# MobilityFirst/gigapaxos

Hardware: AMD Instinct MI355X
Metric: decided_ops_per_sec (higher is better)
Workload: dtype int32; 1 GPU; BASELINE config #3: 1000000 Paxos groups x 3 replicas per GPU, synthetic shuffled accept-reply stream; step = propose_batch(G) + accept_reply_batch(K*G votes), inputs resident in HBM; groups_per_gpu=1000000, groups_total=1000000, replicas=3, rounds_seeded_individually=96, ordered_proposals_promise=True, ordered_batches_mask=1, parallelism=groups sharded across GPUs, no collective on the decide path

## Files before the change

### gigapaxos_amd/csrc/gpx_ar16.hip.h

```cpp
#pragma once
#include "gpx_kernels.hip.h"
#include "gpx_tiles.hip.h"

struct __attribute__((aligned(16))) Vote16 {
  int32_t idx, slot, maxcp;
  uint32_t meta;
};
#define V16_LG_MASK 0x3fffu
#define V16_ESC 0x4000u
#define V16_MAX_SHIFT 10
#define GPX_TL_BUCKET_DYN_MAX (152 * 1024)

struct Stage16 {
  int32_t* base;
  int64_t n;
  __host__ __device__ __forceinline__ int32_t* gidx() const { return base; }
  __host__ __device__ __forceinline__ int32_t* slot() const { return base + n; }
  __host__ __device__ __forceinline__ int32_t* bnum() const { return base + 2 * n; }
  __host__ __device__ __forceinline__ int32_t* bcoord() const { return base + 3 * n; }
  __host__ __device__ __forceinline__ int32_t* median() const { return base + 4 * n; }
  __host__ __device__ __forceinline__ uint8_t* kind() const { return (uint8_t*)(base + 5 * n); }
};
struct VoteCols {
  const int32_t *bnum, *bcoord, *acceptor;
// ... 190 lines not shown
      const bool esc = (meta & V16_ESC) != 0;
      out.bnum = esc ? in.bnum[ix] : b0n;
      out.bcoord = esc ? in.bcoord[ix] : b0c;
    } else {
      out.c = cp;
      if (meta & V16_ESC) {
        out.b = in.acceptor[ix];
        out.bnum = in.bnum[ix];
        out.bcoord = in.bcoord[ix];
      } else {
        out.b = (int32_t)(meta >> 16);
        out.bnum = b0n;
        out.bcoord = b0c;
      }
    }
    done++;
    return true;
  }
  __device__ __forceinline__ void emit(int32_t slot, int32_t x, int32_t y, int32_t z, int32_t kind) {
    if (AC) {
      slot = x;
      z = y;
    }
    if (LDSM) {
      slotA[cur] = slot;
      cpA[cur] = z;
      metaA[cur] = (uint32_t)kind;
      if (nib)
        omask |= 1u << (done - 1);
      else
        keys[nout] = cur;
    } else {
      recG[cur].slot = slot;
      recG[cur].maxcp = z;
      recG[cur].meta = (uint32_t)kind;
      keys[nout] = cur;
    }
    nout++;
  }
  __device__ __forceinline__ void output(int32_t q, int32_t* slot, int32_t* median, int32_t* kind,
                                         uint32_t* om) const {
    uint32_t p;
    if (LDSM && nib) {
      const int d = __ffs((int)*om) - 1;
      *om &= *om - 1;
      p = (uint32_t)start + (uint32_t)stride * (uint32_t)((order >> (4 * d)) & 15ull);
    } else {
      p = (uint32_t)keys[q];
    }
    if (LDSM) {
      *slot = slotA[p];
      *median = cpA[p];
      *kind = (int32_t)metaA[p];
    } else {
      *slot = recG[p].slot;
      *median = recG[p].maxcp;
      *kind = (int32_t)recG[p].meta;
    }
  }
};

__device__ __forceinline__ unsigned long long arrival_order(const int32_t* idxA, int32_t start, int32_t c, int32_t stride = 1) {
  unsigned long long order = 0;
  if (c <= 4) {
    const uint32_t inf = 0xffffffffu;
    const uint32_t i0 = (uint32_t)idxA[start];
    const uint32_t i1 = c > 1 ? (uint32_t)idxA[start + stride] : inf;
    const uint32_t i2 = c > 2 ? (uint32_t)idxA[start + 2 * stride] : inf;
    const uint32_t i3 = c > 3 ? (uint32_t)idxA[start + 3 * stride] : inf;
    const uint32_t r0 = (i1 < i0) + (i2 < i0) + (i3 < i0);
    const uint32_t r1 = (i0 < i1) + (i2 < i1) + (i3 < i1);
    const uint32_t r2 = (i0 < i2) + (i1 < i2) + (i3 < i2);
    const uint32_t r3 = 6u - r0 - r1 - r2;
    const uint32_t o = (1u << (4 * r1)) | (2u << (4 * r2)) | (3u << (4 * r3));
    order = o & 0xffffu;
  } else {
    for (int32_t t = 0; t < c; t++) {
      const uint32_t it = (uint32_t)idxA[start + t * stride];
      int32_t r = 0;
      for (int32_t u = 0; u < c; u++) r += (uint32_t)idxA[start + u * stride] < it;
      order |= (unsigned long long)t << (4 * r);
    }
  }
  return order;
}

#ifdef GPX_AR16_WAVES
#define GPX_AR16_ATTR __attribute__((amdgpu_waves_per_eu(GPX_AR16_WAVES, 8)))
#else
#define GPX_AR16_ATTR
#endif
struct AcceptOut {
  int32_t *r_bnum, *r_bcoord, *r_maxcp;
  uint8_t* r_flags;
  I4* r_packed;
};
#define B16_AR 0
#define B16_ACCEPT 1
#define B16_COMMIT 2
template <int OP, int KMAX, class IT>
__device__ __forceinline__ void ar16_replay_group(const DevState& S, const DevScratch& X, int32_t g, IT& it, CoordPre<KMAX>& P,
                                                  const VoteCols& in, const AcceptOut& R, uint8_t* __restrict__ status,
                                                  const int32_t* idxA, int32_t* slotA, int32_t* cpA, uint32_t* metaA,
                                                  int32_t start, int32_t pstride, int32_t c) {
  auto replay = [&](auto& it_) {
    if (OP == B16_AR)
      apply_ar_group<KMAX>(S, X, g, it_, status, P);
    else if (OP == B16_ACCEPT)
      apply_accept_group(S, X, g, it_, R.r_bnum, R.r_bcoord, R.r_maxcp, R.r_flags, status, R.r_packed);
    else
      apply_commit_group(S, X, g, it_, status);
  };
  if (it.nib) it.order = arrival_order(idxA, start, c, pstride);
  bool fast = false;
  int32_t s0 = 0;
  uint32_t skip = 0;
  int32_t nvote = c;
  bool esc = false;
  if (OP == B16_AR) {
    const bool idle = (P.gf & (GF_EXISTS | GF_STOPPED | GF_HASCOORD)) == GF_EXISTS;
    bool el = c <= 8 && (P.gf & (GF_EXISTS | GF_STOPPED | GF_HASCOORD | GF_PREPARING)) == (GF_EXISTS | GF_HASCOORD) &&
              it.b0n == P.my_bnum && it.b0c == P.my_bcoord;
    if (idle) {
      el = true;
      nvote = 0;
    } else if (el) {
      bool have = false;
      for (int32_t i = 0; i < c; i++) {
        const uint32_t p = (uint32_t)start + (uint32_t)pstride * (uint32_t)((it.order >> (4 * i)) & 15ull);
        if (metaA[p] & V16_ESC) {
          esc = true;
          const int32_t ix = idxA[p];
          const int32_t cmp = ballot_cmp(in.bnum[ix], in.bcoord[ix], P.my_bnum, P.my_bcoord);
          if (cmp < 0) {
            skip |= 1u << i;
            continue;
          }
          el = el && cmp == 0;
        }
        const int32_t sl = slotA[p];
        if (!have) s0 = sl;
        have = true;
        el = el && sl == s0;
      }
      if (have) {
        const int32_t d = jsub(P.next, s0);
        el = el && d >= 1 && d <= S.W;
      }
    }
    fast = __all(el);
  }
  if (fast) {
    if (OP == B16_AR) {
      const int32_t G = S.G, k = (int32_t)GF_K(P.gf);
      int32_t mem[KMAX], ns[KMAX];
#pragma unroll
      for (int j = 0; j < KMAX; j++) {
        mem[j] = (j < k) ? P.mem[j] : 0;
        ns[j] = (j < k) ? P.ns[j] : 0;
      }
      const int64_t off = (int64_t)(s0 & (S.W - 1)) * G + g;
      const uint32_t e0 = (P.have_pe && s0 == jsub(P.next, 1)) ? P.pe : S.p_ring[off];
      uint32_t e = e0;
      int32_t pcount = P.pcount;
      bool ns_dirty = false;
      auto vote = [&](int32_t i, uint32_t p, int32_t acc, int32_t maxcp) {
        int32_t midx = -1;
#pragma unroll
        for (int q = 0; q < KMAX; q++) {
          if (q < k && mem[q] == acc) {
            midx = q;
            if (ns[q] < maxcp) {
              ns[q] = maxcp;
              ns_dirty = true;
            }
          }
        }
        if (e & PR_PRESENT) {
          if (midx >= 0) e |= (1u << midx);
          if (__popc(e & 0xffffu) > k / 2) {
            slotA[p] = s0;
            cpA[p] = median_minus<KMAX>(ns, k);
            metaA[p] = (uint32_t)GPX_D_DECISION;
            it.omask |= 1u << i;
            it.nout++;
            e = 0;
            pcount--;
          }
        }
      };
      if (!__any(esc)) {
        for (int32_t i = 0; i < nvote; i++) {
          const uint32_t p = (uint32_t)start + (uint32_t)pstride * (uint32_t)((it.order >> (4 * i)) & 15ull);
          vote(i, p, (int32_t)(metaA[p] >> 16), cpA[p]);
        }
      } else {
        for (int32_t i = 0; i < nvote; i++) {
          if ((skip >> i) & 1u) continue;
          const uint32_t p = (uint32_t)start + (uint32_t)pstride * (uint32_t)((it.order >> (4 * i)) & 15ull);
          const uint32_t meta = metaA[p];
          vote(i, p, (meta & V16_ESC) ? in.acceptor[idxA[p]] : (int32_t)(meta >> 16), cpA[p]);
        }
      }
      if (e != e0) S.p_ring[off] = e;
      if (ns_dirty) {
#pragma unroll
        for (int q = 0; q < KMAX; q++)
          if (q < k) S.node_slots[(int64_t)q * G + g] = ns[q];
      }
      if (pcount != P.pcount) S.c_pcount[g] = pcount;
    }
  } else {
    replay(it);
  }
}

struct TileLds {
  int32_t* pre;
  uint16_t* st;
};
#define GPX_TILE_LDS_DECL(TILES_)                                   \
  __shared__ int32_t s_pre_[(TILES_) ? GPX_TL_MAXWG + 1 : 1];       \
  __shared__ uint16_t s_st_[(TILES_) ? GPX_TL_MAXWG : 1];           \
  const TileLds TL{s_pre_, s_st_}
template <int OP, int KMAX, bool TILES = false>
__device__ __forceinline__ void bucket16_body(const DevState& S, const DevScratch& X, const Stage16& O, const VoteCols& in,
                                              const AcceptOut& R, uint8_t* __restrict__ status, const TileLds& TL,
                                              const TileArea& A = TileArea{}, int32_t b_in = -1,
                                              const PlaceCols& IP = PlaceCols{}) {
  extern __shared__ __attribute__((aligned(16))) int32_t lds[];
  constexpr bool AC = OP != B16_AR;
  if ((AC || X.gate) && *X.unsorted != X.epoch) return;
  int32_t b = b_in >= 0 ? b_in : (int32_t)blockIdx.x;
  if (TILES && A.xcd_rows && b_in < 0) {
    b = tile_of_block(X.nbk);
    if (b >= X.nbk) return;
  }
  const int32_t gb = X.gb;
  const int32_t l = (int32_t)threadIdx.x;
  int32_t boff, nb;
  int32_t* const s_pre = TL.pre;
  uint16_t* const s_st = TL.st;
  if (TILES) TL_STAMP(4096 + b, 0);
  if (TILES) {
    const unsigned long long* r0 = (const unsigned long long*)A.off + (uint32_t)(b >> 2) * (uint32_t)A.nwg_pad;
    const unsigned long long* r1 = (const unsigned long long*)A.off + (uint32_t)((b + 1) >> 2) * (uint32_t)A.nwg_pad;
    const int32_t per = (A.nwg + gb - 1) >> X.shift;
    int32_t cw[4], ssum = 0, csum = 0;
#pragma unroll
    for (int q = 0; q < 4; q++) {
      const int32_t w = l * per + q;
      cw[q] = 0;
      if (q < per && w < A.nwg) {
        const unsigned long long e0 = r0[w];
        const unsigned long long e1 = ((b & 3) == 3) ? r1[w] : e0;
        const uint16_t o0 = (uint16_t)(e0 >> (16 * (b & 3))), o1 = (uint16_t)(e1 >> (16 * ((b + 1) & 3)));
        const int32_t st = (int32_t)(o0 & 0x7fffu);
        cw[q] = (int32_t)(o1 & 0x7fffu) - st;
        s_st[w] = o0;
        ssum += st;
        csum += cw[q];
      }
    }
    int32_t ex = block_exscan_and_sum_rt(csum, ssum, &nb, &boff);
#pragma unroll
    for (int q = 0; q < 4; q++) {
      const int32_t w = l * per + q;
      if (q < per && w < A.nwg) {
        s_pre[w] = ex;
        ex += cw[q];
      }
    }
    if (l == 0) {
      s_pre[A.nwg] = nb;
      X.bucket_off[b] = boff;
      if (nb == 0) X.bucket_nout[b] = 0;
    }
  } else {
    boff = X.bucket_off[b];
    nb = X.bucket_off[b + 1] - boff;
    if (threadIdx.x == 0) {
      X.bucket_tot[b] = 0;
      if (nb == 0) X.bucket_nout[b] = 0;
    }
  }
  if (nb == 0) return;
  const int32_t g = X.g_base + (b << X.shift) + l;
#ifdef GPX_B16_NOPRELOAD
  const bool pre = false;
#else
  const bool pre = !AC && 2 * nb >= gb;
#endif
  CoordPre<KMAX> P;
  P.have_pe = false;
  P.my_bnum = P.my_bcoord = 0;
  if (pre && g < X.g_end) coord_preload<KMAX>(S, g, P);
  const int32_t L = X.lds_recs;
  int32_t* lcnt = lds;
  int32_t* lcur = lds + gb;
  int32_t* idxA = lds + 2 * gb;
  int32_t* slotA = idxA + L;
  int32_t* cpA = slotA + L;
  uint32_t* metaA = (uint32_t*)(cpA + L);
  const bool in_lds = nb <= L;
  Vote16* recG = (Vote16*)X.rec + boff;
  unsigned long long* keysG = X.perm + boff;
  lcnt[l] = 0;
  const int32_t slot0 = TILES ? A.ref[0] : 0;
  const int32_t ref_bn = TILES ? A.ref[1] : in.bnum[0], ref_bc = TILES ? A.ref[2] : in.bcoord[0];
  int32_t ip_pb = 0, ip_span = -1;
  if (TILES && !AC && IP.div) {
    ip_pb = IP.quot(boff);
    ip_span = IP.quot(boff + nb) - ip_pb;
  }
  int32_t srch = 0;
  if (TILES)
    while ((1 << srch) < A.nwg) srch++;
  auto tile_find = [&](int32_t j) -> int32_t {
    int32_t lo = 0, hi = A.nwg;
    for (int32_t t = 0; t < srch; t++) {
      const int32_t mid = (lo + hi) >> 1;
      const bool up = s_pre[mid] <= j;
      lo = up ? mid : lo;
      hi = up ? hi : mid;
    }
    return lo;
  };
  auto tile_adv = [&](int32_t j, int32_t lo) -> int32_t {
    while (s_pre[lo + 1] <= j) lo++;
    return lo;
  };
  auto tile_pos = [&](int32_t j, int32_t lo, uint32_t* wide) -> uint32_t {
    const uint32_t st = s_st[lo];
    *wide = st & TL_WIDE;
    return __umul24((uint32_t)lo, (uint32_t)A.tile) + (st & 0x7fffu) + (uint32_t)(j - s_pre[lo]);
  };
  auto tile_exp = [&](const Vote8 raw, uint32_t p, uint32_t wide, int32_t lo) -> Vote16 {
    const I4 x = tile_expand(raw, wide ? A.ext + p : (const int2*)nullptr, lo, A.tile, slot0, in.slot, in.maxcp);
    Vote16 v;
    v.idx = x.x, v.slot = x.y, v.maxcp = x.z, v.meta = (uint32_t)x.w;
    return v;
  };
  auto tile_at = [&](int32_t j, int32_t lo) -> Vote16 {
    uint32_t wide;
    const uint32_t p = tile_pos(j, lo, &wide);
    return tile_exp(A.recs[p], p, wide, lo);
  };
  auto tile_rec = [&](int32_t j) -> Vote16 { return tile_at(j, tile_find(j)); };
  if (TILES) __syncthreads();
  if (TILES) TL_STAMP(4096 + b, 1);
#ifdef GPX_ABL_STOP
  if (TILES && GPX_ABL_STOP == 1) return;
#endif
  if (TILES && !in_lds) {
    for (int32_t j = l; j < nb; j += gb) recG[j] = tile_rec(j);
    __threadfence_block();
  }
  __syncthreads();
  Vote16 r0, r1, r2, r3;
  r0.meta = r1.meta = r2.meta = r3.meta = 0;
  r0.idx = r1.idx = r2.idx = r3.idx = 0;
  r0.slot = r1.slot = r2.slot = r3.slot = 0;
  r0.maxcp = r1.maxcp = r2.maxcp = r3.maxcp = 0;
// ... 177 lines not shown
      }
      O.kind()[o] = (uint8_t)kd;
    }
  };
  auto in_place = [&](int32_t tout) -> int32_t {
    if (!TILES || AC || !IP.div) return -1;
    if (tout == ip_span) return ip_pb;
    if (l == 0) A.ref[3] = (int32_t)X.epoch;
    return -1;
  };
  auto put_in_place = [&](int32_t o, int32_t a, int32_t z, int32_t kd) {
    IP.gidx[o] = g;
    IP.slot[o] = a;
    IP.median[o] = z;
    IP.bnum[o] = P.my_bnum;
    IP.bcoord[o] = P.my_bcoord;
    IP.kind[o] = (uint8_t)kd;
  };
  if (in_lds) {
    VoteIter<true, AC> it;
    it.idxA = idxA;
    it.slotA = slotA;
    it.cpA = cpA;
    it.metaA = metaA;
    it.recG = recG;
    it.keys = keysG + start;
    it.in = in;
    it.b0n = ref_bn;
    it.b0c = ref_bc;
    it.start = start;
    it.stride = pstride;
    it.c = c;
    it.done = 0;
    it.nout = 0;
    it.nib = c <= V16_NIB_MAX;
    it.order = 0;
    it.omask = 0;
    it.cur = 0;
    if (live) ar16_replay_group<OP, KMAX>(S, X, g, it, P, in, R, status, idxA, slotA, cpA, metaA, start, pstride, c);
    nout = it.nout;
    omask = it.omask;
    if (TILES) TL_STAMP(4096 + b, 4);
#ifdef GPX_ABL_STOP
    if (TILES && GPX_ABL_STOP == 3) return;
#endif
    int32_t tout;
    const int32_t ex = block_exscan_rt(nout, &tout);
    const int32_t pb = in_place(tout);
    for (int32_t q = 0; q < nout; q++) {
      int32_t sl, md, kd;
      it.output(q, &sl, &md, &kd, &omask);
      put((int64_t)boff + ex + q, sl, md, kd);
      if (pb >= 0) put_in_place(pb + ex + q, sl, md, kd);
    }
    if (l == 0) X.bucket_nout[b] = tout;
    if (TILES) TL_STAMP(4096 + b, 5);
  } else {
    VoteIter<false, AC> it;
    it.idxA = idxA;
    it.slotA = slotA;
    it.cpA = cpA;
    it.metaA = metaA;
    it.recG = recG;
    it.keys = keysG + start;
    it.in = in;
    it.b0n = ref_bn;
    it.b0c = ref_bc;
    it.start = start;
    it.stride = 1;
    it.c = c;
    it.done = 0;
    it.nout = 0;
    it.nib = false;
    it.order = 0;
    it.omask = 0;
    it.cur = 0;
    if (live) replay(it);
    nout = it.nout;
    int32_t tout;
    const int32_t ex = block_exscan_rt(nout, &tout);
    const int32_t pb = in_place(tout);
    for (int32_t q = 0; q < nout; q++) {
      int32_t sl, md, kd;
      it.output(q, &sl, &md, &kd, &omask);
      put((int64_t)boff + ex + q, sl, md, kd);
      if (pb >= 0) put_in_place(pb + ex + q, sl, md, kd);
    }
    if (l == 0) X.bucket_nout[b] = tout;
  }
}

template <int OP, int KMAX>
__global__ __launch_bounds__(1024) GPX_AR16_ATTR void k_bucket16(DevState S, DevScratch X, Stage16 O, VoteCols in,
                                                   AcceptOut R, uint8_t* __restrict__ status) {
  GPX_TILE_LDS_DECL(false);
  bucket16_body<OP, KMAX>(S, X, O, in, R, status, TL);
}
struct TilesKernArgs {
  DevState S;
  DevScratch X;
  Stage16 O;
  VoteCols in;
  uint8_t* status;
  TileArea A;
  PlaceCols IP;
};
static_assert(alignof(DevState) == 8 && alignof(DevScratch) == 8 && alignof(Stage16) == 8 && alignof(VoteCols) == 8 &&
                  alignof(TileArea) == 8 && alignof(PlaceCols) == 8,
              "kernarg layout");
static_assert(sizeof(DevState) % 8 == 0 && sizeof(DevScratch) % 8 == 0 && sizeof(Stage16) % 8 == 0 && sizeof(VoteCols) % 8 == 0 &&
                  sizeof(TileArea) % 8 == 0 && sizeof(PlaceCols) % 8 == 0,
              "kernarg layout");
#ifndef GPX_LAZY
#define GPX_LAZY 7
#endif
template <bool LAZY, class T>
__device__ __forceinline__ const T& lazy_pick(const T& from_kernarg, const T& by_value) {
  if constexpr (LAZY) return from_kernarg;
  else return by_value;
}
#define GPX_TILES_KERNEL_BODY(KM)                                                                                          \
  GPX_TILE_LDS_DECL(true);                                                                                                 \
  const TilesKernArgs* ka = (const TilesKernArgs*)__builtin_amdgcn_kernarg_segment_ptr();                                  \
  bucket16_body<B16_AR, KM, true>(lazy_pick<(GPX_LAZY & 16) != 0>(ka->S, S), lazy_pick<(GPX_LAZY & 2) != 0>(ka->X, X), O,  \
                                  lazy_pick<(GPX_LAZY & 1) != 0>(ka->in, in), AcceptOut{},                                 \
                                  (GPX_LAZY & 8) ? ka->status : status, TL, lazy_pick<(GPX_LAZY & 32) != 0>(ka->A, A), -1, \
                                  lazy_pick<(GPX_LAZY & 4) != 0>(ka->IP, IP))
template <int KMAX>
__global__ __launch_bounds__(1024) GPX_AR16_ATTR void k_bucket_ar16_tiles(DevState S, DevScratch X, Stage16 O, VoteCols in,
                                                                         uint8_t* __restrict__ status, TileArea A, PlaceCols IP) {
  GPX_TILES_KERNEL_BODY(KMAX);
}
#ifndef GPX_K4_WAVES
#define GPX_K4_WAVES 6
#endif
__global__ __launch_bounds__(1024) __attribute__((amdgpu_waves_per_eu(GPX_K4_WAVES, 8))) void k_bucket_ar16_tiles_k4(
    DevState S, DevScratch X, Stage16 O, VoteCols in, uint8_t* __restrict__ status, TileArea A, PlaceCols IP) {
  GPX_TILES_KERNEL_BODY(4);
}
__global__ __launch_bounds__(1024) __attribute__((amdgpu_waves_per_eu(6, 8))) void k_bucket_ar16_tiles_k5(
    DevState S, DevScratch X, Stage16 O, VoteCols in, uint8_t* __restrict__ status, TileArea A, PlaceCols IP) {
  GPX_TILES_KERNEL_BODY(5);
}
__global__ __launch_bounds__(1024) __attribute__((amdgpu_waves_per_eu(6, 8))) void k_bucket_ar16_k5(
    DevState S, DevScratch X, Stage16 O, VoteCols in, AcceptOut R, uint8_t* __restrict__ status) {
  GPX_TILE_LDS_DECL(false);
  bucket16_body<B16_AR, 5>(S, X, O, in, R, status, TL);
}

__global__ __launch_bounds__(GPX_BLOCK) void k_emit_dec16(
    DevScratch X, Stage16 O, int32_t* __restrict__ d_gidx, int32_t* __restrict__ d_slot,
    int32_t* __restrict__ d_bnum, int32_t* __restrict__ d_bcoord, int32_t* __restrict__ d_median,
    uint8_t* __restrict__ d_kind, int32_t* total_out, unsigned long long* acc, const int32_t* base_in,
    int32_t* chain_out, int32_t* in_place = nullptr, int32_t nvotes = 0, const int32_t* __restrict__ c_bnum = nullptr,
    const int32_t* __restrict__ c_bcoord = nullptr) {
  if (X.gate && *X.unsorted != X.epoch) return;
  const bool placed = in_place && in_place[3] != (int32_t)X.epoch;
  if (placed && blockIdx.x != gridDim.x - 1) return;
  const int32_t base0 = base_in ? *base_in : 0;
  const int32_t b = blockIdx.x;
  int32_t before = 0;
  for (int32_t t = threadIdx.x; t < b; t += GPX_BLOCK) before += X.bucket_nout[t];
  int32_t pre;
  block_exscan(before, &pre);
  const int32_t out0 = base0 + pre;
  if (b == (int32_t)gridDim.x - 1 && threadIdx.x == 0) {
    const int32_t tot = pre + X.bucket_nout[b];
    if (total_out) *total_out = base0 + tot;
    if (chain_out) *chain_out = base0 + tot;
    if (acc) atomicAdd(acc, (unsigned long long)tot);
    if (in_place && !placed && tot > 0 && nvotes % tot == 0 && nvotes / tot <= 64 && X.xabort)
      __hip_atomic_store(X.xabort + GPX_IP_LEARN_WORD, (uint32_t)(nvotes / tot), __ATOMIC_RELAXED, __HIP_MEMORY_SCOPE_SYSTEM);
    if (in_place) in_place[placed ? 5 : 6]++;
  }
  if (placed) return;
  const int32_t nd = X.bucket_nout[blockIdx.x];
  const int64_t src = X.bucket_off[blockIdx.x];
  if (threadIdx.x == 0) X.bucket_tot[blockIdx.x] = 0;
  for (int32_t t = threadIdx.x; t < nd; t += GPX_BLOCK) {
    const int32_t g = O.gidx()[src + t];
    d_gidx[out0 + t] = g;
    d_slot[out0 + t] = O.slot()[src + t];
    d_bnum[out0 + t] = c_bnum ? c_bnum[g] : O.bnum()[src + t];
    d_bcoord[out0 + t] = c_bnum ? c_bcoord[g] : O.bcoord()[src + t];
    d_median[out0 + t] = O.median()[src + t];
    d_kind[out0 + t] = O.kind()[src + t];
  }
}

__global__ __launch_bounds__(GPX_BLOCK) void k_emit_runs16(DevScratch X, Stage16 O, int32_t* __restrict__ x_gidx,
                                                          int32_t* __restrict__ x_first,
                                                          int32_t* __restrict__ x_count, int32_t* total_out) {
  if (*X.unsorted != X.epoch) return;
  const int32_t out0 = emit_base(X, total_out, nullptr);
  const int32_t nd = X.bucket_nout[blockIdx.x];
  const int64_t src = X.bucket_off[blockIdx.x];
  for (int32_t t = threadIdx.x; t < nd; t += GPX_BLOCK) {
    x_gidx[out0 + t] = O.gidx()[src + t];
    x_first[out0 + t] = O.slot()[src + t];
    x_count[out0 + t] = O.median()[src + t];
  }
}

__global__ __launch_bounds__(GPX_BLOCK) void k_unpack_replies(DevScratch X, int32_t n, const I4* __restrict__ rows,
                                                             int32_t* __restrict__ r_bnum,
                                                             int32_t* __restrict__ r_bcoord,
                                                             int32_t* __restrict__ r_maxcp,
                                                             uint8_t* __restrict__ r_flags) {
  if (*X.unsorted != X.epoch) return;
  const int32_t i = blockIdx.x * GPX_BLOCK + threadIdx.x;
  if (i >= n) return;
  const I4 r = rows[i];
  r_bnum[i] = r.x;
  r_bcoord[i] = r.y;
  r_maxcp[i] = r.z;
  r_flags[i] = (uint8_t)r.w;
}
```

### gigapaxos_amd/csrc/gpx_elect.hip.h

```cpp
#pragma once

struct PReplyIn {
  const int32_t* pv_off;
  int32_t pv_total;
  const int32_t *pv_slot, *pv_bnum, *pv_bcoord;
  const int64_t* pv_handle;
  const uint8_t* pv_flags;
};
struct PReplyOut {
  int32_t n;
  uint8_t* v_kind;
  int32_t *e_count, *e_median, *e_slot;
  uint8_t* e_kind;
  int64_t* e_handle;
  uint8_t* e_flags;
  uint8_t* status;
};

__global__ __launch_bounds__(GPX_BLOCK) void k_election_begin(DevState S, int32_t n,
                                                             const int32_t* __restrict__ gidx,
                                                             const int32_t* __restrict__ bnum,
                                                             uint8_t* __restrict__ e_status) {
  const int32_t i = blockIdx.x * GPX_BLOCK + threadIdx.x;
  if (i >= n) return;
  const int32_t g = gidx[i];
  if ((uint32_t)g >= (uint32_t)S.G || !(S.g_flags[g] & GF_EXISTS)) {
    e_status[i] = 255;
    return;
  }
  const uint32_t gf = S.g_flags[g];
  const int32_t k = (int32_t)GF_K(gf);
  const bool has = (gf & GF_HASCOORD) != 0;
  const int32_t cmp = has ? ballot_cmp(S.c_bnum[g], S.c_bcoord[g], bnum[i], S.my_id) : -1;
  if (!has || cmp < 0) {
    S.c_bnum[g] = bnum[i];
    S.c_bcoord[g] = S.my_id;
    S.c_next[g] = S.a_slot[g];
    S.c_pcount[g] = 0;
    S.c_wait[g] = 0;
    for (int32_t j = 0; j < k; j++) S.node_slots[(int64_t)j * S.G + g] = -1;
    for (int32_t w = 0; w < S.W; w++) {
      const int64_t o = (int64_t)w * S.G + g;
      S.p_ring[o] = 0;
      S.co_ring[o] = I4{0, 0, 0, 0};
    }
    if (bnum[i] == 0) {
      S.g_flags[g] = (gf | GF_HASCOORD) & ~GF_PREPARING;
      e_status[i] = GPX_EB_ACTIVE;
    } else {
      S.g_flags[g] = gf | GF_HASCOORD | GF_PREPARING;
      e_status[i] = GPX_EB_PREPARING;
    }
  } else if (cmp == 0 && (gf & GF_PREPARING)) {
    e_status[i] = GPX_EB_RESEND;
  } else {
    e_status[i] = GPX_EB_UNCHANGED;
  }
}

template <int KMAX>
__global__ __launch_bounds__(GPX_BLOCK) void k_poke_scan(DevState S, int32_t n,
                                                        const int32_t* __restrict__ gidx,
                                                        uint8_t* __restrict__ poke,
                                                        int32_t* __restrict__ slot,
                                                        int32_t* __restrict__ bnum,
                                                        int32_t* __restrict__ bcoord,
                                                        int32_t* __restrict__ median_cp,
                                                        uint8_t* __restrict__ p_flags,
                                                        uint32_t* __restrict__ heard,
                                                        uint8_t* __restrict__ status) {
  const int32_t i = blockIdx.x * GPX_BLOCK + threadIdx.x;
  if (i >= n) return;
  const int32_t g = gidx ? gidx[i] : i;
  uint8_t pk = GPX_POKE_NONE, fl = 0, st = GPX_S_OK;
  int32_t sl = 0, bn = 0, bc = 0, med = 0;
  uint32_t hd = 0;
  if ((uint32_t)g >= (uint32_t)S.G || !(S.g_flags[g] & GF_EXISTS)) {
    st = GPX_S_NOGROUP;
  } else {
    const uint32_t gf = S.g_flags[g];
    if (gf & GF_HASCOORD) {
      const int32_t s = S.a_slot[g];
      if (gf & GF_PREPARING) {
        pk = GPX_POKE_PREPARE;
        hd = S.c_wait[g];
      } else {
        const int32_t d = jsub(S.c_next[g], s);
        const uint32_t e = (d >= 1 && d <= S.W) ? S.p_ring[(int64_t)(s & (S.W - 1)) * S.G + g] : 0u;
        if (e & PR_PRESENT) {
          const int32_t k = (int32_t)GF_K(gf);
          int32_t ns[KMAX];
#pragma unroll
          for (int q = 0; q < KMAX; q++) ns[q] = (q < k) ? S.node_slots[(int64_t)q * S.G + g] : 0;
          pk = GPX_POKE_ACCEPT;
          med = median_minus<KMAX>(ns, k);
          fl = (e & PR_STOP) ? GPX_PV_STOP : 0;
          hd = e & 0xffffu;
        }
      }
      if (pk != GPX_POKE_NONE) {
        sl = s;
        bn = S.c_bnum[g];
        bc = S.c_bcoord[g];
      }
    }
  }
  poke[i] = pk;
  slot[i] = sl;
  bnum[i] = bn;
  bcoord[i] = bc;
  median_cp[i] = med;
  p_flags[i] = fl;
  heard[i] = hd;
  status[i] = st;
}

#define FE_PRESENT 0x1000u
#define FE_STOP 0x1u
#define FE_KIND(e) (((e) >> 4) & 0xfu)
#define FE_MAKE(kind, stop) (FE_PRESENT | ((uint32_t)(kind) << 4) | ((stop) ? FE_STOP : 0u))

template <class F>
__device__ __forceinline__ void for_signed_order(int32_t lo, int32_t cnt, F f) {
  if (cnt <= 0) return;
  const int32_t hi = (int32_t)((uint32_t)lo + (uint32_t)(cnt - 1));
  int32_t split = 0;
  if (hi < lo) split = (int32_t)(0x80000000u - (uint32_t)lo);
  for (int32_t j = split; j < cnt; j++) f(j);
  for (int32_t j = 0; j < split; j++) f(j);
}

#ifdef GPX_ELECT_BOUNDS
#define EI(i) elect_idx((int32_t)(i), WMAX, __LINE__)
__device__ __forceinline__ int32_t elect_idx(int32_t i, int32_t lim, int line) {
  if ((uint32_t)i >= (uint32_t)lim) {
    printf("elect_group: index %d outside [0, %d) at gpx_elect.hip.h:%d\n", i, lim, line);
    __builtin_trap();
  }
  return i;
}
#else
#define EI(i) (i)
#endif
template <int KMAX, int WMAX>
#ifdef GPX_ELECT_NOINLINE
#define GPX_ELECT_INLINE __attribute__((noinline))
#else
#define GPX_ELECT_INLINE __forceinline__
#endif
__device__ GPX_ELECT_INLINE void elect_group(const DevState& S, const DevScratch& X, int32_t g,
                                         GroupIter& it, const PReplyIn& I, const PReplyOut& O) {
  const int32_t G = S.G, W = S.W, Wm = W - 1, n = O.n;
  uint32_t gf = S.g_flags[g];
  const uint32_t gf0 = gf;
  const bool exists = (gf & GF_EXISTS) != 0;
  const int32_t k = (int32_t)GF_K(gf);
  const bool had = exists && (gf & GF_HASCOORD);
  const int32_t my_bnum = had ? S.c_bnum[g] : 0, my_bcoord = had ? S.c_bcoord[g] : 0;
  int32_t next = had ? S.c_next[g] : 0, pcount = had ? S.c_pcount[g] : 0;
  uint32_t wait = (had && (gf & GF_PREPARING)) ? S.c_wait[g] : 0u;
  int32_t mem[KMAX], ns[KMAX];
#pragma unroll
  for (int q = 0; q < KMAX; q++) {
    mem[q] = (had && q < k) ? S.members[(int64_t)q * G + g] : 0;
    ns[q] = (had && q < k) ? S.node_slots[(int64_t)q * G + g] : 0;
  }
  bool ns_dirty = false, wait_dirty = false, prop_dirty = false;
  int32_t cs[WMAX], cb[WMAX], cc[WMAX], cf[WMAX];
  int64_t ch[WMAX];
  bool co_loaded = false;
  unsigned long long cmask = 0, co_dirty = 0;
  unsigned long long n_drop = 0;

  auto list_preactives = [&](int32_t ix) -> int32_t {
    int32_t cnt = 0;
    const int32_t lo = jsub(next, pcount);
    for_signed_order(lo, pcount, [&](int32_t j) {
      const int32_t s = (int32_t)((uint32_t)lo + (uint32_t)j);
      const int64_t o = (int64_t)(s & Wm) * G + g;
      const uint32_t pe = S.p_ring[o];
      const int64_t q = (int64_t)cnt * n + ix;
      O.e_slot[q] = s;
      O.e_kind[q] = GPX_E_PREACTIVE;
      O.e_handle[q] = S.p_handle[o];
      O.e_flags[q] = (pe & PR_STOP) ? GPX_PV_STOP : 0;
      cnt++;
    });
    return cnt;
  };

  Rec r;
  while (it.next(r)) {
    const int32_t ix = r.idx, acceptor = r.a, first = r.b;
    uint8_t vk = GPX_V_IGNORED;
    int32_t ecount = 0, emed = 0;
    if (!exists) {
      O.status[ix] = GPX_S_NOGROUP;
      n_drop++;
    } else if ((gf & GF_HASCOORD) && (gf & GF_PREPARING)) {
      const int32_t cmp = ballot_cmp(r.bnum, r.bcoord, my_bnum, my_bcoord);
      if (cmp > 0) {
        ecount = list_preactives(ix);
        for (int32_t d = 1; d <= pcount; d++) S.p_ring[(int64_t)(jsub(next, d) & Wm) * G + g] = 0;
        pcount = 0;
        prop_dirty = true;
        gf &= ~(GF_HASCOORD | GF_PREPARING);
        vk = GPX_V_PREEMPTED;
      } else if (cmp == 0) {
        int32_t midx = -1;
#pragma unroll
        for (int q = 0; q < KMAX; q++)
          if (q < k && mem[q] == acceptor) midx = q;
        if (midx >= 0 && !((wait >> midx) & 1u)) {
          if (!co_loaded) {
            for (int32_t w = 0; w < W; w++) {
              const I4 v = S.co_ring[(int64_t)w * G + g];
              cs[EI(w)] = v.x;
              cb[EI(w)] = v.y;
              cc[EI(w)] = v.z;
              cf[EI(w)] = v.w;
              ch[EI(w)] = S.co_handle[(int64_t)w * G + g];
              if (v.w & CO_PRESENT) cmask |= 1ull << w;
            }
            co_loaded = true;
          }
          const int32_t o = I.pv_off[ix], m = I.pv_off[ix + 1] - o;
          bool clash = o < 0 || m < 0 || (int64_t)o + m > (int64_t)I.pv_total;
          if (!clash) {
            int32_t claimed[WMAX];
            unsigned long long nm = 0;
            for (int32_t j = 0; j < m; j++) {
              const int32_t s = I.pv_slot[o + j], x = s & Wm;
              if ((nm >> x) & 1ull) {
                if (claimed[EI(x)] != s) clash = true;
              } else if (((cmask >> x) & 1ull) && cs[EI(x)] != s) {
                clash = true;
              }
              claimed[EI(x)] = s;
              nm |= 1ull << x;
            }
          }
          if (clash) {
            O.status[ix] = GPX_S_WINDOW;
            n_drop++;
          } else {
            vk = GPX_V_RECORDED;
            int32_t ms = first;
            for (int32_t j = 0; j < m; j++) {
              const int32_t s = I.pv_slot[o + j];
              if (jsub(s, ms) < 0) ms = s;
            }
#pragma unroll
            for (int q = 0; q < KMAX; q++)
              if (q < k && mem[q] == acceptor && jsub(ns[q], ms) < 0) {
                ns[q] = ms;
                ns_dirty = true;
              }
            for (int32_t j = 0; j < m; j++) {
              const int32_t s = I.pv_slot[o + j], x = s & Wm;
              const int32_t bn = I.pv_bnum[o + j], bc = I.pv_bcoord[o + j];
              if (!((cmask >> x) & 1ull) || ballot_cmp(bn, bc, cb[EI(x)], cc[EI(x)]) > 0) {
                cs[EI(x)] = s;
                cb[EI(x)] = bn;
                cc[EI(x)] = bc;
                cf[EI(x)] = CO_PRESENT | (I.pv_flags ? (int32_t)(I.pv_flags[o + j] & (GPX_PV_STOP | GPX_PV_NOOP)) : 0);
                ch[EI(x)] = I.pv_handle ? I.pv_handle[o + j] : 0;
                cmask |= 1ull << x;
                co_dirty |= 1ull << x;
              }
            }
            wait |= 1u << midx;
            wait_dirty = true;
            if (__popc(wait & 0xffffu) > k / 2) {
              uint32_t fe[WMAX];
              int64_t fh[WMAX];
              bool fits = true;
              int32_t lo = jsub(next, pcount), pos = pcount;
              if (cmask == 0) {
                ecount = list_preactives(ix);
              } else {
                int32_t maxCarry = 0, maxMin = ns[0];
                bool any = false;
                for (int32_t w = 0; w < W; w++)
                  if ((cmask >> w) & 1ull) {
                    if (!any || jsub(cs[EI(w)], maxCarry) > 0) maxCarry = cs[EI(w)];
                    any = true;
                  }
#pragma unroll
                for (int q = 0; q < KMAX; q++)
                  if (q < k && jsub(ns[q], maxMin) > 0) maxMin = ns[q];
                const int32_t R = jsub(maxCarry, maxMin);
                if (R >= W || R == INT32_MIN) {
                  fits = false;
                } else {
                  const int32_t pre_lo = jsub(next, pcount);
                  unsigned long long removed = 0;
                  bool stop_exists = false, last_stop = false;
                  lo = R >= 0 ? maxMin : (int32_t)((uint32_t)maxCarry + 1u);
                  pos = 0;
                  for (int32_t j = 0; j <= R; j++) {
                    const int32_t cur = (int32_t)((uint32_t)maxMin + (uint32_t)j), x = cur & Wm;
                    const int32_t d = jsub(cur, pre_lo);
                    uint32_t en = 0;
                    int64_t hn = 0;
                    if (((cmask >> x) & 1ull) && cs[EI(x)] == cur) {
                      en = FE_MAKE(GPX_E_CARRY, cf[EI(x)] & GPX_PV_STOP);
                      hn = ch[EI(x)];
                    } else if (!(d >= 0 && d < pcount)) {
                      en = FE_MAKE(GPX_E_NOOP, 0);
                    } else {
                      const int64_t po = (int64_t)x * G + g;
                      const uint32_t pe = S.p_ring[po];
                      const int64_t ph = S.p_handle[po];
                      bool dup = false;
                      for (int32_t w = 0; w < W; w++) dup |= ((cmask >> w) & 1ull) && ch[EI(w)] == ph;
                      if (!dup) {
                        en = FE_MAKE(GPX_E_PREACTIVE, pe & PR_STOP);
                        hn = ph;
                      }
                      removed |= 1ull << d;
                    }
                    fe[EI(pos)] = en;
                    fh[EI(pos)] = hn;
                    if (en & FE_PRESENT) {
                      stop_exists |= (en & FE_STOP) != 0;
                    }
                    last_stop = (en & FE_PRESENT) && (en & FE_STOP);
                    pos++;
                  }
                  auto append = [&](uint32_t en, int64_t hn) {
                    if (pos > 0 && last_stop) return;
                    if (pos < W) {
                      fe[EI(pos)] = en;
                      fh[EI(pos)] = hn;
                    }
                    pos++;
                    stop_exists |= (en & FE_STOP) != 0;
                    last_stop = (en & FE_STOP) != 0;
                  };
                  for_signed_order(pre_lo, pcount, [&](int32_t dd) {
                    if ((removed >> dd) & 1ull) return;
                    const int32_t s = (int32_t)((uint32_t)pre_lo + (uint32_t)dd);
                    const int64_t po = (int64_t)(s & Wm) * G + g;
                    append(FE_MAKE(GPX_E_PREACTIVE, S.p_ring[po] & PR_STOP), S.p_handle[po]);
                  });
                  if (stop_exists && pos > 0 && !last_stop) append(FE_MAKE(GPX_E_NEWSTOP, 1), 0);
                  fits = pos <= W;
                  if (fits) {
                    for (int32_t d = 1; d <= pcount; d++) S.p_ring[(int64_t)(jsub(next, d) & Wm) * G + g] = 0;
                    int32_t live = 0;
                    for (int32_t j = 0; j < pos; j++)
                      if (fe[EI(j)] & FE_PRESENT) {
                        const int32_t s = (int32_t)((uint32_t)lo + (uint32_t)j);
                        S.p_ring[(int64_t)(s & Wm) * G + g] = PR_PRESENT | ((fe[EI(j)] & FE_STOP) ? PR_STOP : 0u);
                        live++;
                      }
                    next = (int32_t)((uint32_t)lo + (uint32_t)pos);
                    pcount = live;
                    prop_dirty = true;
                    for_signed_order(lo, pos, [&](int32_t j) {
                      if (!(fe[EI(j)] & FE_PRESENT)) return;
                      const int64_t q = (int64_t)ecount * n + ix;
                      O.e_slot[q] = (int32_t)((uint32_t)lo + (uint32_t)j);
                      O.e_kind[q] = (uint8_t)FE_KIND(fe[EI(j)]);
                      O.e_handle[q] = fh[EI(j)];
                      O.e_flags[q] = (fe[EI(j)] & FE_STOP) ? GPX_PV_STOP : 0;
                      ecount++;
                    });
                  }
                }
              }
              if (fits) {
                emed = median_minus<KMAX>(ns, k);
                gf &= ~GF_PREPARING;
                vk = GPX_V_ELECTED;
              } else {
                O.status[ix] = GPX_S_WINDOW;
                n_drop++;
              }
            }
          }
        }
      }
    }
    O.v_kind[ix] = vk;
    O.e_count[ix] = ecount;
    O.e_median[ix] = emed;
  }
  if (co_dirty) {
    for (int32_t w = 0; w < W; w++)
      if ((co_dirty >> w) & 1ull) {
        S.co_ring[(int64_t)w * G + g] = I4{cs[EI(w)], cb[EI(w)], cc[EI(w)], cf[EI(w)]};
        S.co_handle[(int64_t)w * G + g] = ch[EI(w)];
      }
  }
  if (ns_dirty) {
#pragma unroll
    for (int q = 0; q < KMAX; q++)
      if (q < k) S.node_slots[(int64_t)q * G + g] = ns[q];
  }
  if (wait_dirty) S.c_wait[g] = wait;
  if (prop_dirty) {
    S.c_next[g] = next;
    S.c_pcount[g] = pcount;
  }
  if (gf != gf0) S.g_flags[g] = gf;
  if (n_drop) atomicAdd(&X.counters[2], n_drop);
}

template <int KMAX, int WMAX>
__global__ __launch_bounds__(1024) void k_bucket_prepare_reply(DevState S, DevScratch X, PReplyIn I,
                                                               PReplyOut O) {
  extern __shared__ __attribute__((aligned(16))) int32_t lds[];
  BucketView bv;
  if (!bucket_prepare(X, lds, &bv, []() {})) return;
  const int32_t g0 = blockIdx.x << X.shift;
  for (int32_t l = threadIdx.x; l < X.gb; l += (int32_t)blockDim.x) {
    const int32_t c = bv.lcnt[l];
    const int32_t g = g0 + l;
    if (c == 0 || g >= S.G) continue;
    GroupIter it;
    it.init(bv, l, c);
    elect_group<KMAX, WMAX>(S, X, g, it, I, O);
  }
}
```

### gigapaxos_amd/csrc/gpx_engine.hip

```cpp
#include <hip/hip_runtime.h>
#include <unistd.h>
#include <dirent.h>
#include <signal.h>
#include <sys/stat.h>
#include <sys/types.h>
#include <cerrno>
#include <chrono>

#include <cmath>
#include <cstdio>
#include <cstdlib>
#include <cstring>
#include <map>
#include <mutex>
#include <string>
#include <vector>
#include <algorithm>
#include <cassert>
#include <initializer_list>

#include "gpx_kernels.hip.h"
#include "gpx_ar16.hip.h"
#include "gpx_direct.hip.h"
#include "gpx_one.hip.h"
// ... 413 lines not shown
    LAUNCH_F(e, "k_hist", k_hist<true>, tile_grid(nsuper), lds, n, ntiles, gidx, e->S.G, e->X, status,
             is_votes, check_order, hsub);
  else
    LAUNCH_F(e, "k_hist", k_hist<false>, tile_grid(nsuper), lds, n, ntiles, gidx, e->S.G, e->X, status,
             is_votes, check_order, hsub);
}

void launch_scatter_ac(gpx_engine* e, int32_t n, const int32_t* gidx, const int32_t* bnum,
                       const int32_t* bcoord, const int32_t* slot, const int32_t* median_cp,
                       const uint8_t* flags, int32_t* r_bnum, int32_t* r_bcoord, int32_t* r_maxcp,
                       uint8_t* r_flags, int32_t only_unsorted = 0) {
  const int ntiles = ntiles_for(n);
  const bool vec = aligned16({gidx, bnum, bcoord, slot, median_cp}) && !((uintptr_t)flags & 3);
  if (vec)
    LAUNCH_F(e, "k_scatter_ac", k_scatter_ac<true>, tile_grid(ntiles), (size_t)e->X.nbk * 4, n, ntiles,
             e->S.G, e->X, gidx, bnum, bcoord, slot, median_cp, flags, r_bnum, r_bcoord, r_maxcp, r_flags,
             only_unsorted);
  else
    LAUNCH_F(e, "k_scatter_ac", k_scatter_ac<false>, tile_grid(ntiles), (size_t)e->X.nbk * 4, n, ntiles,
             e->S.G, e->X, gidx, bnum, bcoord, slot, median_cp, flags, r_bnum, r_bcoord, r_maxcp, r_flags,
             only_unsorted);
}

int check_batch(gpx_engine* h, int32_t n) {
  if (!h || n < 0) return GPX_EINVAL;
  if (n > h->cfg.max_batch) return GPX_ECAPACITY;
  if (h->h_abort && *(volatile uint32_t*)h->h_abort) {
    snprintf(g_err, sizeof(g_err), "an exchange kernel gave up waiting for its grid (call epoch %u): engine state is "
             "incomplete; set GPX_DEVICE_SHARERS to the number of processes sharing the device", *(volatile uint32_t*)h->h_abort);
    return GPX_EDEVICE;
  }
  return GPX_OK;
}

#define SYNC_CHECKED(h, stream_)                                \
  do {                                                          \
    HIPCHK(hipStreamSynchronize(stream_));                      \
    if (int _rc_abort = check_batch((h), 0)) return _rc_abort;  \
  } while (0)

int xchg_share(const gpx_engine* e) {
  std::lock_guard<std::mutex> lk(g_live_mu);
  int live = 1;
  auto it = g_live_streams.find(e->device);
  if (it != g_live_streams.end()) live = std::max<int>(1, (int)it->second.size());
  if (e->sharers_set) return live * e->sharers;
  return live + proc_registry_foreign(e->device);
}
bool xchg_ctl(gpx_engine* e, int nchunks, GridXchg* Q, int* grid, const void* kernel, int block) {
  const int g16 = (std::max(nchunks, 1) + GPX_GX_LINES - 1) / GPX_GX_LINES * GPX_GX_LINES;
  if (!e->one_launch) return false;
  int per_cu = 2;
  {
    auto it = e->occ.find(kernel);
    if (it == e->occ.end()) {
      int nb = 0;
      if (hipOccupancyMaxActiveBlocksPerMultiprocessor(&nb, kernel, block, 0) != hipSuccess) {
        (void)hipGetLastError();
        nb = 0;
      }
      it = e->occ.emplace(kernel, nb).first;
    }
    per_cu = std::min(2, it->second - 1);
  }
  if (per_cu < 1 || (int64_t)g16 * xchg_share(e) > (int64_t)per_cu * e->cus) return false;
  const OneCtl C = one_ctl(e);
  *grid = g16;
  Q->arrive = (uint32_t*)(e->one_words + GPX_ONE_TICKETS);
  Q->verdict = C.verdict;
  Q->epoch = C.epoch;
  e->gx_arrive += (uint32_t)(g16 / GPX_GX_LINES);
  Q->arrive_target = e->gx_arrive + e->xchg_test_skew;
  Q->timeout_ms = e->xchg_timeout_ms;
  return true;
}

constexpr size_t GPX_PAGEABLE_PIECE = (size_t)512 << 10;
bool host_is_pinned(gpx_engine* e, const void* p) {
  for (auto& r : e->registered)
    if ((const char*)p >= r.first && (const char*)p < r.first + r.second) return true;
  hipPointerAttribute_t at{};
  if (hipPointerGetAttributes(&at, p) != hipSuccess) {
    (void)hipGetLastError();
    return false;
  }
  return at.type == hipMemoryTypeHost;
}
hipError_t xfer(gpx_engine* e, void* dst, const void* src, size_t bytes, hipMemcpyKind kind, hipStream_t st) {
  if (bytes <= GPX_PAGEABLE_PIECE || host_is_pinned(e, kind == hipMemcpyHostToDevice ? src : (const void*)dst))
    return hipMemcpyAsync(dst, src, bytes, kind, st);
  for (size_t o = 0; o < bytes; o += GPX_PAGEABLE_PIECE) {
    const hipError_t rc = hipMemcpyAsync((char*)dst + o, (const char*)src + o, std::min(GPX_PAGEABLE_PIECE, bytes - o), kind, st);
    if (rc != hipSuccess) return rc;
  }
  return hipSuccess;
}

template <int KMAX>
void launch_bucket_ar16(gpx_engine* e, const Stage16& O, const VoteCols& in, uint8_t* status) {
  LAUNCH_B(e, "k_bucket_ar16", (k_bucket16<B16_AR, KMAX>), e->S, e->X, O, in, AcceptOut{}, status);
}
template <int KMAX>
void launch_bucket_propose(gpx_engine* e, int32_t* slot, int32_t* bnum, int32_t* bcoord,
                           int32_t* median, uint8_t* status, const int64_t* handle) {
  LAUNCH_B(e, "k_bucket_propose", (k_bucket_propose<KMAX>), e->S, e->X, slot, bnum, bcoord, median,
           status, handle);
}

struct Stage {
  gpx_engine* e;
  size_t in_off = 0, out_off = 0;
  explicit Stage(gpx_engine* e_) : e(e_) {}
  static size_t a16(size_t b) { return (b + 15) & ~(size_t)15; }
  template <typename T>
  const T* in(const T* host, size_t count) {
    if (!host) return nullptr;
    const size_t b = count * sizeof(T);
    memcpy(e->hs_in + in_off, host, b);
    const T* d = (const T*)(e->ds_in + in_off);
    in_off += a16(b);
    return d;
  }
  template <typename T>
  T* out(size_t count, const T** host_view) {
    T* d = (T*)(e->ds_out + out_off);
    *host_view = (const T*)(e->hs_out + out_off);
    out_off += a16(count * sizeof(T));
    return d;
  }
  int upload() {
    if (in_off) HIPCHK(hipMemcpyAsync(e->ds_in, e->hs_in, in_off, hipMemcpyHostToDevice, e->sF));
    return GPX_OK;
  }
  int finish() {
    HIPCHK(hipMemcpyAsync(e->hs_out, e->ds_out, out_off, hipMemcpyDeviceToHost, e->sB));
    HIPCHK(hipStreamSynchronize(e->sB));
    return check_batch(e, 0);
  }
};

}

extern "C" {

int gpx_abi_version(void) { return GPX_ABI_VERSION; }
const char* gpx_last_error(void) { return g_err; }

int gpx_engine_create(const gpx_config* cfg, gpx_engine** out) {
  g_err[0] = 0;
  if (!cfg || !out) return GPX_EINVAL;
  if (cfg->max_groups <= 0 || cfg->kmax < 1 || cfg->kmax > GPX_KMAX_LIMIT || cfg->max_batch <= 0)
    return GPX_EINVAL;
  if (cfg->window < 4 || cfg->window > 64 || (cfg->window & (cfg->window - 1))) return GPX_EINVAL;
  int ndev = 0;
  hipError_t de = hipErrorNoDevice;
  const int attempts = access("/dev/kfd", F_OK) == 0 ? 15 : 1;
  for (int attempt = 0; attempt < attempts; attempt++) {
    de = hipGetDeviceCount(&ndev);
    if (de == hipSuccess && ndev > 0) break;
    (void)hipGetLastError();
    if (de != hipErrorNoDevice && de != hipSuccess) break;
    if (attempt + 1 < attempts) usleep(200 * 1000);
  }
  if (de != hipSuccess || ndev <= 0) {
    snprintf(g_err, sizeof(g_err), "no HIP device visible (%s)", de == hipSuccess ? "count 0" : hipGetErrorString(de));
    return GPX_EDEVICE;
  }
  gpx_engine* e = new gpx_engine();
  e->cfg = *cfg;
#define HIPCHK_CREATE(expr)                                                                  \
  do {                                                                                       \
    hipError_t _e = (expr);                                                                  \
    if (_e != hipSuccess) {                                                                  \
      snprintf(g_err, sizeof(g_err), "%s:%d %s -> %s", __FILE__, __LINE__, #expr,            \
               hipGetErrorString(_e));                                                       \
      gpx_engine_destroy(e);                                                                 \
      return GPX_EDEVICE;                                                                    \
    }                                                                                        \
  } while (0)
  if (cfg->device >= 0) {
    HIPCHK_CREATE(hipSetDevice(cfg->device));
    e->device = cfg->device;
  } else {
    HIPCHK_CREATE(hipGetDevice(&e->device));
  }
  HIPCHK_CREATE(hipStreamCreateWithFlags(&e->own_stream, hipStreamNonBlocking));
  apply_streams(e);
  const size_t G = (size_t)cfg->max_groups, W = (size_t)cfg->window, K = (size_t)cfg->kmax;
  const size_t N = (size_t)cfg->max_batch;
  DevState& S = e->S;
  S.G = cfg->max_groups;
  S.kmax = cfg->kmax;
  S.W = cfg->window;
  S.my_id = cfg->my_id;
  S.flags = cfg->flags;
  int rc = GPX_OK;
#define A(ptr, count, zero)                                   \
  if ((rc = dev_alloc(e, &(ptr), (count), (zero))) != GPX_OK) { \
    gpx_engine_destroy(e);                                    \
    return rc;                                                \
  }
  A(S.g_flags, G, true);
  A(S.g_version, G, true);
  A(S.a_slot, G, true);
  A(S.a_bnum, G, true);
  A(S.a_bcoord, G, true);
  A(S.a_gc, G, true);
  A(S.c_bnum, G, true);
  A(S.c_bcoord, G, true);
  A(S.c_next, G, true);
  A(S.c_pcount, G, true);
  A(S.members, K * G, true);
  A(S.node_slots, K * G, true);
  A(S.p_ring, W * G, true);
  A(S.acc_ring, W * G, true);
  A(S.com_ring, W * G, true);
  DevScratch& X = e->X;
  auto nbk_for = [&](int sh) { return (int64_t)((G + ((size_t)1 << sh) - 1) >> sh); };
  X.shift = nbk_for(GPX_MIN_SHIFT + 1) >= 256 ? GPX_MIN_SHIFT + 1 : GPX_MIN_SHIFT;
  while (nbk_for(X.shift) > GPX_MAX_BUCKETS) X.shift++;
  if (const char* sh = getenv("GPX_BUCKET_SHIFT")) {
    const int v = atoi(sh);
    if (v >= GPX_MIN_SHIFT && v <= 20 && nbk_for(v) <= GPX_MAX_BUCKETS) X.shift = v;
  }
  X.gb = 1 << X.shift;
  X.nbk = (int32_t)nbk_for(X.shift);
  X.g_base = 0;
  X.g_end = cfg->max_groups;
  e->bucket_threads = std::min(1024, X.gb);
  {
    int64_t want = (int64_t)cfg->kmax * X.gb;
    want += want / 4 + 64;
    if (cfg->kmax <= 3 && X.gb == 256) want = 960;
    const int64_t lds_cap = ((int64_t)160 * 1024 - 1024 - (int64_t)X.gb * 8) / (8 + 4 * GPX_PAY_WORDS);
    want = std::min<int64_t>(want, std::min<int64_t>(lds_cap, (int64_t)GPX_BUCKET_ITEMS * e->bucket_threads));
    if (const char* lr = getenv("GPX_LDS_RECS")) want = std::min<int64_t>(want, std::max(64, atoi(lr)));
    X.lds_recs = (int32_t)want;
    e->lds_recs_max = X.lds_recs;
    e->lds_recs_hw = (int32_t)std::max<int64_t>(want, std::min<int64_t>(lds_cap, (int64_t)GPX_BUCKET_ITEMS * e->bucket_threads));
  }
  {
    const int64_t cap16 = ((int64_t)160 * 1024 - 1024 - (int64_t)X.gb * 8) / 16;
    int64_t want = (int64_t)cfg->kmax * X.gb;
    want += want / 4 + 128;
    e->lds16_max = (int32_t)std::min<int64_t>(want, cap16);
    e->lds16_hw = (int32_t)cap16;
    e->ac16 = X.shift <= V16_MAX_SHIFT && e->bucket_threads == X.gb;
    if (X.shift <= V16_MAX_SHIFT) {
      e->shift16 = X.shift;
      e->nbk16 = X.nbk;
      e->ar_passes = 1;
    } else {
      e->shift16 = V16_MAX_SHIFT;
      const int64_t range = (int64_t)GPX_MAX_BUCKETS << V16_MAX_SHIFT;
      e->ar_passes = (int32_t)(((int64_t)G + range - 1) / range);
      e->nbk16 = GPX_MAX_BUCKETS;
      const int64_t gb16 = (int64_t)1 << V16_MAX_SHIFT;
      const int64_t cap16b = ((int64_t)160 * 1024 - 1024 - gb16 * 8) / 16;
      int64_t want16 = (int64_t)cfg->kmax * gb16;
      want16 += want16 / 4 + 128;
      e->lds16_max = (int32_t)std::min<int64_t>(want16, cap16b);
      e->lds16_hw = (int32_t)cap16b;
    }
    if ((rc = dev_alloc(e, &e->ar_chain, 2, true)) != GPX_OK) {
      gpx_engine_destroy(e);
      return rc;
    }
  }
  if (const char* lp = getenv("GPX_LDS_PAD")) e->lds_pad = (size_t)std::max(0, atoi(lp));
  if (const char* tr = getenv("GPX_TRY_RUNS")) e->env_mask = atoi(tr) ? GPX_TRY_REPLY_RUNS : 0;
  e->ar_tiles = true;
  if (const char* sl = getenv("GPX_AR_TILES")) e->ar_tiles = atoi(sl) != 0;
  if (const char* sl = getenv("GPX_AR_INPLACE")) e->ar_in_place = atoi(sl) != 0;
  if (const char* tt = getenv("GPX_TILE_T")) e->tile_force = atoi(tt);
  if (const char* tt = getenv("GPX_TILE_NT")) e->tile_threads = atoi(tt);
  e->tile_area.xcd_rows = 1;
  if (const char* xr = getenv("GPX_TILE_XCD_ROWS")) e->tile_area.xcd_rows = atoi(xr) != 0;
#ifdef GPX_TL_TRACE
  if (const char* ab = getenv("GPX_TL_ABLATE")) e->tile_area.xcd_rows |= atoi(ab) << 1;
#endif
  if (const char* sv = getenv("GPX_SAR_MAX_N")) e->sar_max_n = std::max(0, std::min(GPX_SAR_MAX_N, atoi(sv)));
  e->sar_max_n = std::min(e->sar_max_n, cfg->max_batch);
  e->ordered_mask = e->env_mask;
  e->bucket_lds = GPX_BUCKET_LDS_BYTES(X.gb, X.lds_recs) + e->lds_pad;
  const size_t bucket_lds_hw = GPX_BUCKET_LDS_BYTES(X.gb, e->lds_recs_hw) + e->lds_pad;
  if (bucket_lds_hw > 64 * 1024) {
    const void* fns[] = {(const void*)k_bucket_propose<4>,
                         (const void*)k_bucket_propose<8>, (const void*)k_bucket_propose<16>,
                         (const void*)k_bucket_accept,     (const void*)k_bucket_commit,
                         (const void*)k_bucket_pack_ar,    (const void*)k_bucket_reqbatch,
                         (const void*)k_bucket_prepare,
                         (const void*)k_bucket_prepare_reply<4, 64>,
                         (const void*)k_bucket_prepare_reply<8, 64>,
                         (const void*)k_bucket_prepare_reply<16, 64>};
    for (const void* f : fns)
      HIPCHK_CREATE(hipFuncSetAttribute(f, hipFuncAttributeMaxDynamicSharedMemorySize, (int)bucket_lds_hw));
  }
  {
    if ((rc = dev_alloc(e, &e->small_tickets, 2 * (GPX_SMALL_DIRECT_MAX_N / GPX_DCHUNK), true)) != GPX_OK ||
        (rc = dev_alloc(e, &e->small_draw, 1, true)) != GPX_OK) {
      gpx_engine_destroy(e);
      return rc;
    }
    if (hipHostMalloc((void**)&e->hs_in, GPX_STAGE_BYTES, hipHostMallocDefault) != hipSuccess ||
        hipHostMalloc((void**)&e->hs_out, GPX_STAGE_BYTES, hipHostMallocDefault) != hipSuccess) {
      snprintf(g_err, sizeof(g_err), "hipHostMalloc(%zu) failed", (size_t)GPX_STAGE_BYTES);
      gpx_engine_destroy(e);
      return GPX_ENOMEM;
    }
    if ((rc = dev_alloc(e, &e->ds_in, GPX_STAGE_BYTES, false)) != GPX_OK ||
        (rc = dev_alloc(e, &e->ds_out, GPX_STAGE_BYTES, false)) != GPX_OK) {
      gpx_engine_destroy(e);
      return rc;
    }
  }
  {
    const size_t hw16 = GPX_BUCKET16_LDS_BYTES((size_t)1 << e->shift16, e->lds16_hw) + e->lds_pad;
    const void* fns[] = {(const void*)k_bucket16<B16_AR, 4>, (const void*)k_bucket_ar16_k5, (const void*)k_bucket16<B16_AR, 8>,
                         (const void*)k_bucket16<B16_AR, 16>, (const void*)k_bucket16<B16_ACCEPT, 4>,
                         (const void*)k_bucket16<B16_COMMIT, 4>};
    for (const void* f : fns)
      HIPCHK_CREATE(hipFuncSetAttribute(f, hipFuncAttributeMaxDynamicSharedMemorySize, (int)hw16));
  }
  {
    const void* fns[] = {(const void*)k_ar_tiny<4>, (const void*)k_ar_tiny<8>, (const void*)k_ar_tiny<16>};
    for (const void* f : fns)
      HIPCHK_CREATE(hipFuncSetAttribute(f, hipFuncAttributeMaxDynamicSharedMemorySize, (int)GPX_SAR_LDS_BYTES));
  }
  {
    const int hl = GPX_HSUB_MAX * std::max(X.nbk, e->nbk16) * (int)sizeof(int32_t);
    if (hl > 64 * 1024) {
      HIPCHK_CREATE(hipFuncSetAttribute((const void*)k_hist<true>, hipFuncAttributeMaxDynamicSharedMemorySize, hl));
      HIPCHK_CREATE(hipFuncSetAttribute((const void*)k_hist<false>, hipFuncAttributeMaxDynamicSharedMemorySize, hl));
    }
  }
  const size_t nbk_alloc = (size_t)std::max(X.nbk, e->nbk16);
  for (auto& f : e->fs) {
    A(f.bucket_tot, nbk_alloc, true);
    A(f.tile_rel, ((N + GPX_TILE - 1) / GPX_TILE) * nbk_alloc, false);
    A(f.bucket_off, nbk_alloc + 1, true);
    A(f.rec, N, false);
    A(f.unsorted, 1, true);
    A(f.chunk_cnt, GPX_CHUNK_CNT_WORDS(N), true);
  }
  X.bucket_tot = e->fs[0].bucket_tot;
  X.tile_rel = e->fs[0].tile_rel;
  X.bucket_off = e->fs[0].bucket_off;
  X.rec = e->fs[0].rec;
  X.unsorted = e->fs[0].unsorted;
  X.epoch = 1;
  A(X.rank2, N, false);
  A(X.perm, N, false);
  A(X.o_rec, N, false);
  A(X.bucket_nout, nbk_alloc, true);
  A(e->rec_tag, N, true);
  A(e->one_words, GPX_ONE_TICKETS + GPX_GX_LINES * 16, true);
  A(X.counters, 3, true);
  for (int i = 0; i < 12; i++) A(e->st_i32[i], N, false);
  for (int i = 0; i < 4; i++) A(e->st_u8[i], N, false);
  A(e->st_count, 4, true);
#undef A
  {
    HIPCHK_CREATE(hipDeviceGetAttribute(&e->cus, hipDeviceAttributeMultiprocessorCount, e->device));
    if (const char* sv = getenv("GPX_XCHG_SLOTS")) e->one_launch = atoi(sv) != 0;
// ... 246 lines not shown
  {
    LaunchScope _ls(e, "k_route_scatter");
    hipLaunchKernelGGL(k_route_scatter, dim3(ntiles), dim3(GPX_ROUTE_NT), 0, e->stream, n, n_groups_global, n_shards,
                       C, g2l, (const int32_t*)e->route_cnt, (const int32_t*)shard_off);
  }
  HIPCHK(hipGetLastError());
  return GPX_OK;
}


struct TileShape {
  int32_t T, NT;
};
#ifdef GPX_TL_TRACE
static unsigned long long* tl_trace_dev = nullptr;
static void tl_trace_begin(gpx_engine* e) {
  if (!tl_trace_dev) {
    HIPQ(hipMalloc(&tl_trace_dev, TL_TRACE_ROWS * 8 * sizeof(unsigned long long)));
    HIPQ(hipMemcpyToSymbol(HIP_SYMBOL(g_tl_trace), &tl_trace_dev, sizeof(tl_trace_dev)));
  }
  HIPQ(hipMemsetAsync(tl_trace_dev, 0, TL_TRACE_ROWS * 8 * sizeof(unsigned long long), e->stream));
}
static void tl_trace_end(gpx_engine* e) {
  const char* tf = getenv("GPX_TL_TRACE_FILE");
  if (!tf) return;
  HIPQ(hipStreamSynchronize(e->stream));
  std::vector<unsigned long long> tr((size_t)TL_TRACE_ROWS * 8);
  HIPQ(hipMemcpy(tr.data(), tl_trace_dev, tr.size() * 8, hipMemcpyDeviceToHost));
  if (FILE* fp = fopen(tf, "wb")) {
    fwrite(tr.data(), 8, tr.size(), fp);
    fclose(fp);
  }
}
#endif
static TileShape tile_shape(const gpx_engine* e, int32_t n, int32_t nbk) {
  if (e->tile_force) return TileShape{e->tile_force, e->tile_threads ? e->tile_threads : (e->tile_force <= 8192 ? 512 : 1024)};
  const int64_t cus = std::max(1, e->cus);
  static const struct { TileShape s; int64_t round_ns; } cand[] = {{{12288, 1024}, 27900}, {{8192, 1024}, 17300}, {{4096, 512}, 10000}};
  TileShape best = cand[2].s;
  int64_t best_cost = INT64_MAX;
  for (const auto& c : cand) {
    if (GPX_TL_LDS_BYTES(nbk, c.s.T, c.s.NT) > (size_t)158 * 1024) continue;
    const int64_t nwg = ((int64_t)n + c.s.T - 1) / c.s.T;
    if (nwg > GPX_TL_MAXWG) continue;
    const int64_t cost = (nwg + cus - 1) / cus * c.round_ns + nwg * 5;
    if (cost < best_cost) best_cost = cost, best = c.s;
  }
  return best;
}
static bool ar_tiles_call(gpx_engine* e, int32_t n, const int32_t* gidx, const int32_t* bnum, const int32_t* bcoord,
                          const int32_t* slot, const int32_t* acceptor, const int32_t* max_cp, int32_t* d_gidx,
                          int32_t* d_slot, int32_t* d_bnum, int32_t* d_bcoord, int32_t* d_median_cp, uint8_t* d_kind,
                          int32_t* n_out, uint8_t* status) {
  const int32_t nbk = e->nbk16;
  if (nbk > GPX_MAX_BUCKETS || e->shift16 > 10 || e->shift16 < 8) return false;
  TileShape ts = tile_shape(e, n, nbk);
  if (nbk + 1 > ts.NT * 8) ts.NT = 1024;
  assert(nbk + 1 <= ts.NT * 8);
  const int32_t T = ts.T;
  if ((T != 4096 && T != 8192 && T != 12288 && T != 16384) || (ts.NT != 512 && ts.NT != 1024) || T % (ts.NT * 4)) return false;
  const int r4 = T / (ts.NT * 4);
  if (!(ts.NT == 1024 && r4 >= 1 && r4 <= 4) && !(ts.NT == 512 && (r4 == 2 || r4 == 4))) return false;
  if (GPX_TL_LDS_BYTES(nbk, T, ts.NT) > (size_t)158 * 1024) return false;
  const int32_t nwg = (n + T - 1) / T;
  if (nwg > GPX_TL_MAXWG) return false;
  const size_t N = (size_t)e->cfg.max_batch;
  TileArea& A = e->tile_area;
  if (!A.recs) {
    const size_t cap = (N + 4095) / 4096 * 4096 + 16384;
    const size_t nwg_max = std::min<size_t>((N + 4095) / 4096, GPX_TL_MAXWG);
    const size_t pad = (nwg_max + 7) / 8 * 8;
    if (dev_alloc(e, &A.recs, cap, false) != GPX_OK || dev_alloc(e, &A.ext, cap, false) != GPX_OK ||
        dev_alloc(e, &A.off, ((size_t)nbk / 4 + 2) * pad * 4, true) != GPX_OK || dev_alloc(e, &A.ref, 8, true) != GPX_OK) {
      A.recs = nullptr;
      e->ar_tiles = false;
      return false;
    }
    A.nwg_pad = (int32_t)pad;
    const int maxlds = (int)std::min<size_t>(GPX_TL_LDS_BYTES(nbk, 16384, 1024), (size_t)158 * 1024);
    HIPQ(hipFuncSetAttribute((const void*)k_scatter_tiles<1024, 4>, hipFuncAttributeMaxDynamicSharedMemorySize, maxlds));
    HIPQ(hipFuncSetAttribute((const void*)k_scatter_tiles<1024, 3>, hipFuncAttributeMaxDynamicSharedMemorySize, maxlds));
    HIPQ(hipFuncSetAttribute((const void*)k_scatter_tiles<1024, 2>, hipFuncAttributeMaxDynamicSharedMemorySize, maxlds));
    HIPQ(hipFuncSetAttribute((const void*)k_scatter_tiles<1024, 1>, hipFuncAttributeMaxDynamicSharedMemorySize, maxlds));
    HIPQ(hipFuncSetAttribute((const void*)k_scatter_tiles<512, 4>, hipFuncAttributeMaxDynamicSharedMemorySize, maxlds));
    HIPQ(hipFuncSetAttribute((const void*)k_scatter_tiles<512, 2>, hipFuncAttributeMaxDynamicSharedMemorySize, maxlds));
    const size_t hw16 = std::min<size_t>(GPX_BUCKET16_LDS_BYTES((size_t)1 << e->shift16, e->lds16_hw) + e->lds_pad,
                                         (size_t)GPX_TL_BUCKET_DYN_MAX);
    HIPQ(hipFuncSetAttribute((const void*)k_bucket_ar16_tiles_k4, hipFuncAttributeMaxDynamicSharedMemorySize, (int)hw16));
    HIPQ(hipFuncSetAttribute((const void*)k_bucket_ar16_tiles_k5, hipFuncAttributeMaxDynamicSharedMemorySize, (int)hw16));
    HIPQ(hipFuncSetAttribute((const void*)k_bucket_ar16_tiles<8>, hipFuncAttributeMaxDynamicSharedMemorySize, (int)hw16));
    HIPQ(hipFuncSetAttribute((const void*)k_bucket_ar16_tiles<16>, hipFuncAttributeMaxDynamicSharedMemorySize, (int)hw16));
  }
  A.nwg = nwg;
  A.tile = T;
  const DevScratch X0 = e->X;
  const int threads0 = e->bucket_threads;
  e->X.shift = e->shift16;
  e->X.gb = 1 << e->shift16;
  e->X.nbk = nbk;
  e->bucket_threads = e->X.gb;
  begin_back(e, 0, n, true);
  {
    const int32_t kslot = e->cfg.kmax <= 4 ? 4 : 8;
    if ((int64_t)n / nbk >= e->X.gb / 4 && e->X.lds_recs < kslot * e->X.gb) {
      e->X.lds_recs = kslot * e->X.gb;
      e->bucket_lds = GPX_BUCKET16_LDS_BYTES(e->X.gb, e->X.lds_recs) + e->lds_pad;
    }
  }
  if (e->bucket_lds > (size_t)GPX_TL_BUCKET_DYN_MAX) {
    e->X.lds_recs = (int32_t)(((size_t)GPX_TL_BUCKET_DYN_MAX - e->lds_pad - (size_t)e->X.gb * 8) / 16);
    e->bucket_lds = GPX_BUCKET16_LDS_BYTES(e->X.gb, e->X.lds_recs) + e->lds_pad;
  }
  const size_t lds = GPX_TL_LDS_BYTES(nbk, T, ts.NT);
#ifdef GPX_TL_TRACE
  tl_trace_begin(e);
#endif
  {
    LaunchScope _ls(e, "k_scatter_tiles");
#define GPX_LAUNCH_TILES(NT_, R4_)                                                                                       \
  hipLaunchKernelGGL(HIP_KERNEL_NAME(k_scatter_tiles<NT_, R4_>), dim3(tile_grid(A.nwg)), dim3(NT_), lds, e->stream, n, e->S.G, \
                     e->X, A, gidx, bnum, bcoord, slot, acceptor, max_cp, status)
    if (ts.NT == 1024 && r4 == 4) GPX_LAUNCH_TILES(1024, 4);
    else if (ts.NT == 1024 && r4 == 3) GPX_LAUNCH_TILES(1024, 3);
    else if (ts.NT == 1024 && r4 == 2) GPX_LAUNCH_TILES(1024, 2);
    else if (ts.NT == 1024 && r4 == 1) GPX_LAUNCH_TILES(1024, 1);
    else if (ts.NT == 512 && r4 == 4) GPX_LAUNCH_TILES(512, 4);
    else if (ts.NT == 512 && r4 == 2) GPX_LAUNCH_TILES(512, 2);
    else assert(!"k_scatter_tiles: no instantiation for this shape (refused above)");
#undef GPX_LAUNCH_TILES
  }
  const Stage16 O{(int32_t*)e->X.o_rec, (int64_t)N};
  const VoteCols in{bnum, bcoord, acceptor, slot, max_cp};
  int32_t ip_div = 0;
  if (e->ar_in_place && n < (1 << 26)) {
    const uint32_t learnt = e->h_abort ? ((volatile uint32_t*)e->h_abort)[GPX_IP_LEARN_WORD] : 0u;
    ip_div = learnt >= 1 && learnt <= 64 ? (int32_t)learnt : std::max(1, e->cfg.kmax);
  }
  const PlaceCols IP{d_gidx, d_slot, d_bnum, d_bcoord, d_median_cp, d_kind, ip_div,
                     ip_div > 1 ? (uint32_t)((1ull << 32) / (uint64_t)ip_div) + 1u : 0u};
  {
    LaunchScope _ls(e, e->cfg.kmax <= 4 ? "k_bucket_ar16_tiles_k4" : e->cfg.kmax <= 5 ? "k_bucket_ar16_tiles_k5" : "k_bucket_ar16_tiles");
    const dim3 grid(A.xcd_rows ? tile_grid(nbk) : nbk), block(e->bucket_threads);
    if (e->cfg.kmax <= 4)
      hipLaunchKernelGGL(k_bucket_ar16_tiles_k4, grid, block, e->bucket_lds, e->stream, e->S, e->X, O, in, status, A, IP);
    else if (e->cfg.kmax <= 5)
      hipLaunchKernelGGL(k_bucket_ar16_tiles_k5, grid, block, e->bucket_lds, e->stream, e->S, e->X, O, in, status, A, IP);
    else if (e->cfg.kmax <= 8)
      hipLaunchKernelGGL(k_bucket_ar16_tiles<8>, grid, block, e->bucket_lds, e->stream, e->S, e->X, O, in, status, A, IP);
    else
      hipLaunchKernelGGL(k_bucket_ar16_tiles<16>, grid, block, e->bucket_lds, e->stream, e->S, e->X, O, in, status, A, IP);
  }
  LAUNCH(e, "k_emit_dec16", k_emit_dec16, e->X.nbk, e->X, O, d_gidx, d_slot, d_bnum, d_bcoord, d_median_cp, d_kind, n_out,
         &e->X.counters[1], (const int32_t*)nullptr, (int32_t*)nullptr, ip_div ? A.ref : (int32_t*)nullptr, n,
         ip_div ? (const int32_t*)e->S.c_bnum : (const int32_t*)nullptr, (const int32_t*)e->S.c_bcoord);
#ifdef GPX_TL_TRACE
  tl_trace_end(e);
#endif
  const int32_t lds_recs = e->X.lds_recs;
  const int32_t gate = e->X.gate;
  e->X = X0;
  e->X.lds_recs = lds_recs;
  e->X.gate = gate;
  e->bucket_threads = threads0;
  return true;
}

static void ar_partition(gpx_engine* e, int32_t n, const int32_t* gidx, const int32_t* bnum, const int32_t* bcoord,
                         const int32_t* slot, const int32_t* acceptor, const int32_t* max_cp, int32_t* d_gidx,
                         int32_t* d_slot, int32_t* d_bnum, int32_t* d_bcoord, int32_t* d_median_cp,
                         uint8_t* d_kind, int32_t* n_out, uint8_t* status) {
  const int ntiles = ntiles_for(n);
  const bool vec = aligned16({gidx, bnum, bcoord, slot, acceptor, max_cp});
  const DevScratch X0 = e->X;
  const int threads0 = e->bucket_threads;
  const int64_t NB = ((int64_t)e->S.G + ((int64_t)1 << e->shift16) - 1) >> e->shift16;
  int64_t want_passes = e->ar_passes;
  {
    const double m = (double)n / (double)NB;
    const int64_t pc = (int64_t)((m + 5.0 * sqrt(m)) / (double)e->lds16_hw) + 1;
    want_passes = std::min<int64_t>(NB, std::max<int64_t>(want_passes, pc));
  }
  const int64_t bpp = (NB + want_passes - 1) / want_passes;
  const int32_t passes = (int32_t)((NB + bpp - 1) / bpp);
  if (e->ar_tiles && passes == 1 && vec && ar_tiles_call(e, n, gidx, bnum, bcoord, slot, acceptor, max_cp, d_gidx, d_slot, d_bnum,
                                                        d_bcoord, d_median_cp, d_kind, n_out, status))
    return;
  const size_t N = (size_t)e->cfg.max_batch;
  int32_t* o32 = (int32_t*)e->X.o_rec;
  const Stage16 O{o32, (int64_t)N};
  const VoteCols in{bnum, bcoord, acceptor};
  for (int32_t p = 0; p < passes; p++) {
    e->X.shift = e->shift16;
    e->X.gb = 1 << e->shift16;
    e->X.nbk = e->nbk16;
    e->bucket_threads = e->X.gb;
    if (passes > 1) {
      const int64_t range = bpp << e->shift16;
      e->X.g_base = (int32_t)(p * range);
      e->X.g_end = (int32_t)std::min<int64_t>(e->S.G, (p + 1) * range);
      e->X.nbk = (int32_t)((e->X.g_end - e->X.g_base + e->X.gb - 1) >> e->shift16);
    }
    if (p == 0) begin_back(e, 0, n / passes, true);
    front_hist(e, n, gidx, p == 0 ? status : nullptr, p == 0 ? 1 : -1, e->X.gate ? 2 : 0);
    if (vec)
      LAUNCH_F(e, "k_scatter_ar16", k_scatter_ar16<true>, tile_grid(ntiles), (size_t)e->X.nbk * 4, n,
               ntiles, e->S.G, e->X, gidx, bnum, bcoord, slot, acceptor, max_cp);
    else
      LAUNCH_F(e, "k_scatter_ar16", k_scatter_ar16<false>, tile_grid(ntiles), (size_t)e->X.nbk * 4, n,
               ntiles, e->S.G, e->X, gidx, bnum, bcoord, slot, acceptor, max_cp);
    if (e->cfg.kmax <= 4)
      launch_bucket_ar16<4>(e, O, in, status);
    else if (e->cfg.kmax <= 5)
      LAUNCH_B(e, "k_bucket_ar16", k_bucket_ar16_k5, e->S, e->X, O, in, AcceptOut{}, status);
    else if (e->cfg.kmax <= 8)
      launch_bucket_ar16<8>(e, O, in, status);
    else
      launch_bucket_ar16<16>(e, O, in, status);
    LAUNCH(e, "k_emit_dec16", k_emit_dec16, e->X.nbk, e->X, O, d_gidx, d_slot, d_bnum, d_bcoord,
           d_median_cp, d_kind, n_out, &e->X.counters[1],
           (const int32_t*)(p > 0 ? e->ar_chain + (p & 1) : nullptr),
           passes > 1 ? e->ar_chain + ((p + 1) & 1) : (int32_t*)nullptr);
    const int32_t lds_recs = e->X.lds_recs;
    const int32_t gate = e->X.gate;
    e->X = X0;
    e->X.lds_recs = lds_recs;
    e->X.gate = gate;
    e->bucket_threads = threads0;
  }
}

#ifdef GPX_SAR_TRACE
static unsigned long long* sar_trace_dev = nullptr;
static void sar_trace_begin(gpx_engine* e) {
  if (!sar_trace_dev) {
    HIPQ(hipMalloc(&sar_trace_dev, 256 * 16 * sizeof(unsigned long long)));
    HIPQ(hipMemcpyToSymbol(HIP_SYMBOL(g_sar_trace), &sar_trace_dev, sizeof(sar_trace_dev)));
  }
  HIPQ(hipMemsetAsync(sar_trace_dev, 0, 256 * 16 * sizeof(unsigned long long), e->stream));
}
static void sar_trace_end(gpx_engine* e) {
  const char* tf = getenv("GPX_SAR_TRACE_FILE");
  if (!tf) return;
  HIPQ(hipStreamSynchronize(e->stream));
  std::vector<unsigned long long> tr(256 * 16);
  HIPQ(hipMemcpy(tr.data(), sar_trace_dev, tr.size() * 8, hipMemcpyDeviceToHost));
  if (FILE* fp = fopen(tf, "wb")) {
    fwrite(tr.data(), 8, tr.size(), fp);
    fclose(fp);
  }
}
#endif

int gpx_accept_reply_batch_dev(gpx_engine* h, int32_t n, const int32_t* gidx,
                               const int32_t* bnum, const int32_t* bcoord, const int32_t* slot,
                               const int32_t* acceptor, const int32_t* max_cp, int32_t* d_gidx,
                               int32_t* d_slot, int32_t* d_bnum, int32_t* d_bcoord,
                               int32_t* d_median_cp, uint8_t* d_kind, int32_t* n_out,
                               uint8_t* status) {
  int rc = check_batch(h, n);
  if (rc != GPX_OK) return rc;
  if (n == 0) {
    HIPCHK(hipMemsetAsync(n_out, 0, sizeof(int32_t), h->sB));
    return GPX_OK;
  }
  gpx_engine* e = h;
  const int fs = begin_front(e);
  e->X.gate = 0;
  const bool runs_promised = (e->ordered_mask & GPX_ORDERED_REPLY_RUNS) != 0;
  const bool runs_try = runs_promised || (e->ordered_mask & GPX_TRY_REPLY_RUNS) != 0;
  if (!runs_promised && n <= e->sar_max_n && e->S.G <= GPX_SAR_MAX_G) {
    e->last.kind = 0;
#ifdef GPX_SAR_TRACE
    sar_trace_begin(e);
#endif
    {
      LaunchScope _ls(e, "k_ar_tiny");
#define GPX_LAUNCH_AR_TINY(KM)                                                                                          \
  hipLaunchKernelGGL(k_ar_tiny<KM>, dim3(1), dim3(GPX_SAR_BLOCK), GPX_SAR_LDS_BYTES, e->stream, e->S, e->X, n, gidx, bnum, \
                     bcoord, slot, acceptor, max_cp, d_gidx, d_slot, d_bnum, d_bcoord, d_median_cp, d_kind, n_out, status)
      if (e->cfg.kmax <= 4)
        GPX_LAUNCH_AR_TINY(4);
      else if (e->cfg.kmax <= 8)
        GPX_LAUNCH_AR_TINY(8);
      else
        GPX_LAUNCH_AR_TINY(16);
#undef GPX_LAUNCH_AR_TINY
    }
#ifdef GPX_SAR_TRACE
    sar_trace_end(e);
#endif
    end_call(e, fs);
    HIPCHK(hipGetLastError());
    return GPX_OK;
  }
  if (runs_try) {
    const size_t N = (size_t)e->cfg.max_batch;
    if (!e->runs_info && (rc = dev_alloc(e, &e->runs_info, 2, true)) != GPX_OK) return rc;
    RunsInfo* info = e->runs_info + (e->runs_seq & 1);
    RunsInfo* next_info = e->runs_info + ((e->runs_seq + 1) & 1);
    e->runs_seq++;
    const int nchunks = (n + GPX_DCHUNK - 1) / GPX_DCHUNK;
    const RunsStage st{DecCols{d_gidx, d_slot, d_bnum, d_bcoord, d_median_cp, d_kind}, e->rec_tag, e->fs[0].chunk_cnt,
                       Stage16{(int32_t*)e->X.o_rec, (int64_t)N}};
    const int32_t refuse = runs_promised ? 1 : 0;
    if (!e->runs_arrive &&
        (rc = dev_alloc(e, &e->runs_arrive,
                        (size_t)32 * (3 + N / GPX_RBLOCK / 16 + 1),
// ... 1183 lines not shown

int gpx_group_create(gpx_engine* h, int32_t n, const int32_t* gidx, const int32_t* members,
                     const uint8_t* k, const gpx_hri* rows, uint8_t* status) {
  if (!h || n < 0) return GPX_EINVAL;
  if (n == 0) return GPX_OK;
  if (!gidx || !members || !k || !rows) return GPX_EINVAL;
  const int32_t chunk = 1 << 18;
  int32_t *d_g = nullptr, *d_m = nullptr;
  uint8_t *d_k = nullptr, *d_s = nullptr;
  gpx_hri* d_r = nullptr;
  const int32_t c0 = std::min(n, chunk);
  HIPCHK(hipMalloc((void**)&d_g, (size_t)c0 * 4));
  HIPCHK(hipMalloc((void**)&d_m, (size_t)c0 * 4 * h->cfg.kmax));
  HIPCHK(hipMalloc((void**)&d_k, (size_t)c0));
  HIPCHK(hipMalloc((void**)&d_s, (size_t)c0));
  HIPCHK(hipMalloc((void**)&d_r, (size_t)c0 * sizeof(gpx_hri)));
  int rc = GPX_OK;
  for (int32_t o = 0; o < n && rc == GPX_OK; o += chunk) {
    const int32_t c = std::min(chunk, n - o);
    H2D_B(d_g, gidx + o, (size_t)c * 4);
    H2D_B(d_m, members + (size_t)o * h->cfg.kmax, (size_t)c * 4 * h->cfg.kmax);
    H2D_B(d_k, k + o, (size_t)c);
    H2D_B(d_r, rows + o, (size_t)c * sizeof(gpx_hri));
    LAUNCH(h, "k_group_create", k_group_create, grid_for(c), h->S, c, (const int32_t*)d_g,
           (const int32_t*)d_m, (const uint8_t*)d_k, (const gpx_hri*)d_r, d_s, NameCopies{h->N.rows, (uint8_t*)h->N.tab});
    if (status) D2H(status + o, d_s, (size_t)c);
    HIPCHK(hipStreamSynchronize(h->sB));
    rc = check_batch(h, 0);
  }
  (void)hipFree(d_g);
  (void)hipFree(d_m);
  (void)hipFree(d_k);
  (void)hipFree(d_s);
  (void)hipFree(d_r);
  return rc;
}

static int retire_impl(gpx_engine* h, int32_t n, const int32_t* gidx, int32_t mode, gpx_hri* rows,
                       uint8_t* status) {
  if (!h || n < 0) return GPX_EINVAL;
  if (n == 0) return GPX_OK;
  if (!gidx) return GPX_EINVAL;
  const int32_t chunk = 1 << 18;
  int32_t* d_g = nullptr;
  uint8_t* d_s = nullptr;
  gpx_hri* d_r = nullptr;
  const int32_t c0 = std::min(n, chunk);
  HIPCHK(hipMalloc((void**)&d_g, (size_t)c0 * 4));
  HIPCHK(hipMalloc((void**)&d_s, (size_t)c0));
  HIPCHK(hipMalloc((void**)&d_r, (size_t)c0 * sizeof(gpx_hri)));
  int rc = GPX_OK;
  for (int32_t o = 0; o < n && rc == GPX_OK; o += chunk) {
    const int32_t c = std::min(chunk, n - o);
    H2D_B(d_g, gidx + o, (size_t)c * 4);
    LAUNCH(h, "k_group_retire", k_group_retire, grid_for(c), h->S, c, (const int32_t*)d_g, mode, d_r,
           d_s, NameCopies{h->N.rows, (uint8_t*)h->N.tab});
    if (rows) D2H(rows + o, d_r, (size_t)c * sizeof(gpx_hri));
    if (status) D2H(status + o, d_s, (size_t)c);
    HIPCHK(hipStreamSynchronize(h->sB));
    rc = check_batch(h, 0);
  }
  (void)hipFree(d_g);
  (void)hipFree(d_s);
  (void)hipFree(d_r);
  return rc;
}

int gpx_group_retire(gpx_engine* h, int32_t n, const int32_t* gidx, int32_t mode, gpx_hri* rows,
                     uint8_t* status) {
  if (mode != GPX_RETIRE_PAUSE && mode != GPX_RETIRE_KILL) return GPX_EINVAL;
  return retire_impl(h, n, gidx, mode, rows, status);
}

int gpx_group_snapshot(gpx_engine* h, int32_t n, const int32_t* gidx, gpx_hri* rows,
                       uint8_t* status) {
  if (!rows) return GPX_EINVAL;
  return retire_impl(h, n, gidx, 2, rows, status);
}

int gpx_group_dump(gpx_engine* h, int32_t gidx, int32_t* buf, int32_t cap) {
  if (!h || !buf) return GPX_EINVAL;
  SYNC_CHECKED(h, h->sB);
  std::vector<int32_t> w;
  const DevState& S = h->S;
  auto rd32 = [&](const void* base, int64_t idx, int32_t* out) -> hipError_t {
    return hipMemcpy(out, (const char*)base + idx * 4, 4, hipMemcpyDeviceToHost);
  };
  if (gidx < 0 || gidx >= S.G) {
    if (cap < 1) return GPX_ECAPACITY;
    buf[0] = 0;
    return 1;
  }
  int32_t gf_i = 0;
  HIPCHK(rd32(S.g_flags, gidx, &gf_i));
  const uint32_t gf = (uint32_t)gf_i;
  w.push_back((gf & GF_EXISTS) ? 1 : 0);
  if (gf & GF_EXISTS) {
    const int32_t k = (int32_t)GF_K(gf);
    int32_t v = 0;
    HIPCHK(rd32(S.g_version, gidx, &v));
    w.push_back(v);
    w.push_back(k);
    for (int j = 0; j < k; j++) {
      HIPCHK(rd32(S.members, (int64_t)j * S.G + gidx, &v));
      w.push_back(v);
    }
    const void* accf[4] = {S.a_slot, S.a_bnum, S.a_bcoord, S.a_gc};
    for (auto p : accf) {
      HIPCHK(rd32(p, gidx, &v));
      w.push_back(v);
    }
    w.push_back((gf & GF_STOPPED) ? 1 : 0);
    struct Ent {
      int32_t slot, a, b, c;
      uint8_t f;
    };
    auto read_ring = [&](const I4* ring, int shift, std::vector<Ent>& out) -> int {
      for (int32_t x = 0; x < S.W; x++) {
        I4 fe;
        HIPCHK(hipMemcpy(&fe, S.acc_ring + ((int64_t)x * S.G + gidx), sizeof(I4), hipMemcpyDeviceToHost));
        const uint8_t f = (uint8_t)(((uint32_t)fe.w >> shift) & 0xffu);
        if (!(f & RF_PRESENT)) continue;
        I4 r = fe;
        if (ring != S.acc_ring)
          HIPCHK(hipMemcpy(&r, ring + ((int64_t)x * S.G + gidx), sizeof(I4), hipMemcpyDeviceToHost));
        out.push_back(Ent{r.x, r.y, r.z, r.w, f});
      }
      std::sort(out.begin(), out.end(), [](const Ent& p, const Ent& q) { return p.slot < q.slot; });
      return GPX_OK;
    };
    std::vector<Ent> acc, com;
    int rc = read_ring(S.acc_ring, 0, acc);
    if (rc != GPX_OK) return rc;
    rc = read_ring(S.com_ring, CF_SHIFT, com);
    if (rc != GPX_OK) return rc;
    w.push_back((int32_t)acc.size());
    for (auto& en : acc) {
      w.push_back(en.slot);
      w.push_back(en.a);
      w.push_back(en.b);
      w.push_back((en.f & RF_STOP) ? 1 : 0);
    }
    w.push_back((int32_t)com.size());
    for (auto& en : com) {
      w.push_back(en.slot);
      w.push_back(en.a);
      w.push_back(en.b);
      w.push_back(en.c);
      w.push_back((en.f & RF_HASVALUE) ? 1 : 0);
      w.push_back((en.f & RF_STOP) ? 1 : 0);
    }
    w.push_back((gf & GF_HASCOORD) ? 1 : 0);
    if (gf & GF_HASCOORD) {
      int32_t next = 0;
      HIPCHK(rd32(S.c_bnum, gidx, &v));
      w.push_back(v);
      HIPCHK(rd32(S.c_bcoord, gidx, &v));
      w.push_back(v);
      HIPCHK(rd32(S.c_next, gidx, &next));
      w.push_back(next);
      for (int j = 0; j < k; j++) {
        HIPCHK(rd32(S.node_slots, (int64_t)j * S.G + gidx, &v));
        w.push_back(v);
      }
      std::vector<std::pair<int32_t, uint32_t>> props;
      for (int32_t d = S.W; d >= 1; d--) {
        const int32_t s = (int32_t)((uint32_t)next - (uint32_t)d);
        int32_t ev = 0;
        HIPCHK(rd32(S.p_ring, (int64_t)(s & (S.W - 1)) * S.G + gidx, &ev));
        if ((uint32_t)ev & PR_PRESENT) props.push_back({s, (uint32_t)ev});
      }
      std::sort(props.begin(), props.end(),
                [](const std::pair<int32_t, uint32_t>& p, const std::pair<int32_t, uint32_t>& q) {
                  return p.first < q.first;
                });
      w.push_back((int32_t)props.size());
      for (auto& pr : props) {
        w.push_back(pr.first);
        w.push_back((pr.second & PR_STOP) ? 1 : 0);
        w.push_back((int32_t)(pr.second & 0xffffu));
      }
      const bool preparing = (gf & GF_PREPARING) != 0;
      w.push_back(preparing ? 0 : 1);
      if (preparing) {
        auto rd64 = [&](const int64_t* base, int64_t idx, int64_t* out) -> hipError_t {
          return hipMemcpy(out, base + idx, 8, hipMemcpyDeviceToHost);
        };
        w.push_back(1);
        HIPCHK(rd32(S.c_wait, gidx, &v));
        w.push_back(v);
        for (auto& pr : props) {
          int64_t hv = 0;
          HIPCHK(rd64(S.p_handle, (int64_t)(pr.first & (S.W - 1)) * S.G + gidx, &hv));
          w.push_back((int32_t)(uint32_t)hv);
          w.push_back((int32_t)((uint64_t)hv >> 32));
        }
        struct Co {
          I4 v;
          int64_t hv;
        };
        std::vector<Co> cos;
        for (int32_t x = 0; x < S.W; x++) {
          Co c;
          HIPCHK(hipMemcpy(&c.v, S.co_ring + ((int64_t)x * S.G + gidx), sizeof(I4), hipMemcpyDeviceToHost));
          if (!(c.v.w & CO_PRESENT)) continue;
          HIPCHK(rd64(S.co_handle, (int64_t)x * S.G + gidx, &c.hv));
          cos.push_back(c);
        }
        std::sort(cos.begin(), cos.end(), [](const Co& p, const Co& q) { return p.v.x < q.v.x; });
        w.push_back((int32_t)cos.size());
        for (auto& c : cos) {
          w.push_back(c.v.x);
          w.push_back(c.v.y);
          w.push_back(c.v.z);
          w.push_back(c.v.w & (GPX_PV_STOP | GPX_PV_NOOP));
          w.push_back((int32_t)(uint32_t)c.hv);
          w.push_back((int32_t)((uint64_t)c.hv >> 32));
        }
      }
    }
  }
  if ((int32_t)w.size() > cap) return GPX_ECAPACITY;
  memcpy(buf, w.data(), w.size() * sizeof(int32_t));
  return (int32_t)w.size();
}

}

#include "gpx_wire_host.inc"
#include "gpx_elect_host.inc"
```

### gigapaxos_amd/csrc/gpx_kernels.hip.h

```cpp
#pragma once
#include <hip/hip_runtime.h>
#include <stdint.h>

#include "../../include/gpx.h"

#ifdef GPX_SAR_TRACE
__device__ unsigned long long* g_sar_trace = nullptr;
#define SAR_STAMP(wg, k)                                                                             \
  do {                                                                                               \
    if (threadIdx.x == 0 && g_sar_trace) g_sar_trace[(size_t)(wg) * 16 + (k)] = wall_clock64();        \
  } while (0)
#else
#define SAR_STAMP(wg, k) do { } while (0)
#endif

#ifdef GPX_TL_TRACE
__device__ unsigned long long* g_tl_trace = nullptr;
#define TL_TRACE_ROWS 8192
#define TL_STAMP(row, k)                                                                             \
  do {                                                                                               \
    if (threadIdx.x == 0 && g_tl_trace) g_tl_trace[(size_t)(row) * 8 + (k)] = wall_clock64();          \
  } while (0)
#define TL_CLOCK(row, k)  \
  do {                                                                                               \
    if (threadIdx.x == 0 && g_tl_trace) g_tl_trace[(size_t)(row) * 8 + (k)] = clock64();               \
  } while (0)
#else
#define TL_STAMP(row, k) do { } while (0)
#define TL_CLOCK(row, k) do { } while (0)
#endif

struct __attribute__((aligned(16))) I4 {
  int32_t x, y, z, w;
};
__host__ __device__ __forceinline__ I4 mk4(int32_t x, int32_t y, int32_t z, int32_t w) {
  I4 r;
  r.x = x;
  r.y = y;
  r.z = z;
  r.w = w;
  return r;
}
struct __attribute__((aligned(32))) Rec {
  int32_t idx, lg, a, b, c, bnum, bcoord, pad;
};
struct __attribute__((aligned(32))) Out {
  int32_t gidx, slot, x, y, z, kind, pad0, pad1;
};
__device__ __forceinline__ Out mk_out(int32_t gidx, int32_t slot, int32_t x, int32_t y, int32_t z,
                                      int32_t kind) {
  Out o;
  o.gidx = gidx;
  o.slot = slot;
  o.x = x;
  o.y = y;
  o.z = z;
  o.kind = kind;
  o.pad0 = 0;
  o.pad1 = 0;
  return o;
}

#define GPX_BLOCK 256
#ifndef GPX_FBLOCK
#define GPX_FBLOCK 1024
#endif
#ifndef GPX_TILE
#define GPX_TILE 4096
#endif
#define GPX_HSUB_MAX 8
#define GPX_TILE_ITEMS (GPX_TILE / GPX_FBLOCK)
#define GPX_TILE_VECS (GPX_TILE_ITEMS / 4)
#define GPX_SCAN_ITEMS 8
#define GPX_SCAN_TILE (GPX_FBLOCK * GPX_SCAN_ITEMS)
#define GPX_SMALL_SEG 16
#define GPX_MIN_SHIFT 8
#define GPX_MAX_BUCKETS 4096

#define GF_EXISTS 1u
#define GF_STOPPED 2u
#define GF_HASCOORD 4u
#define GF_PREPARING 8u
#define GF_K(f) (((f) >> 8) & 0xffu)

#define PR_PRESENT 0x10000u
#define PR_STOP 0x20000u
#define RF_PRESENT 1
#define RF_STOP 2
#define RF_HASVALUE 4

struct DevState {
  int32_t G, kmax, W, my_id;
  uint32_t flags;
  uint32_t* g_flags;
  int32_t* g_version;
  int32_t *a_slot, *a_bnum, *a_bcoord, *a_gc;
  int32_t *c_bnum, *c_bcoord, *c_next, *c_pcount;
  int32_t* members;
  int32_t* node_slots;
  uint32_t* p_ring;
  I4* acc_ring;
  I4* com_ring;
  uint32_t* c_wait;
  I4* co_ring;
  int64_t* co_handle;
  int64_t* p_handle;
};
#define CO_PRESENT 0x100

struct DevScratch {
  int32_t shift, nbk, gb;
  int32_t g_base, g_end;
  int32_t lds_recs;
  int32_t* bucket_tot;
  int32_t* tile_rel;
  int32_t* bucket_off;
  Rec* rec;
  int32_t* rank2;
  unsigned long long* perm;
  Out* o_rec;
  int32_t* bucket_nout;
  unsigned long long* counters;
  uint32_t* unsorted;
  uint32_t epoch;
  int32_t gate;
  uint32_t* xabort;
};

#define GPX_XCHG_TIMEOUT_MS 10000u
struct XchgWait {
  uint32_t spins = 0;
  unsigned long long t0 = 0;
  __device__ __forceinline__ bool tired(uint32_t limit_ms) {
    if ((++spins & 1023u) != 0) return false;
    const unsigned long long now = wall_clock64();
    if (!t0) {
      t0 = now;
      return false;
    }
    return now - t0 > (unsigned long long)limit_ms * 100000ull;
  }
};
__device__ __forceinline__ void xchg_abort(const DevScratch& X) {
  if (X.xabort) __hip_atomic_store(X.xabort, X.epoch ? X.epoch : 1u, __ATOMIC_RELAXED, __HIP_MEMORY_SCOPE_SYSTEM);
}

__device__ __forceinline__ int32_t jsub(int32_t a, int32_t b) {
  return (int32_t)((uint32_t)a - (uint32_t)b);
}
__device__ __forceinline__ int32_t ballot_cmp(int32_t n1, int32_t c1, int32_t n2, int32_t c2) {
  return (n1 != n2) ? jsub(n1, n2) : jsub(c1, c2);
}

__device__ __forceinline__ int32_t wave_incscan(int32_t v) {
#ifdef GPX_SCAN_SHFL
  const int lane = threadIdx.x & 63;
  int32_t x = v;
#pragma unroll
  for (int d = 1; d < 64; d <<= 1) {
    int32_t y = __shfl_up(x, d, 64);
    if (lane >= d) x += y;
  }
  return x;
#else
  int32_t x = v;
  x += __builtin_amdgcn_update_dpp(0, x, 0x111, 0xf, 0xf, true);
  x += __builtin_amdgcn_update_dpp(0, x, 0x112, 0xf, 0xf, true);
  x += __builtin_amdgcn_update_dpp(0, x, 0x114, 0xf, 0xf, true);
  x += __builtin_amdgcn_update_dpp(0, x, 0x118, 0xf, 0xf, true);
  x += __builtin_amdgcn_update_dpp(0, x, 0x142, 0xa, 0xf, false);
  x += __builtin_amdgcn_update_dpp(0, x, 0x143, 0xc, 0xf, false);
  return x;
#endif
}
__device__ __forceinline__ int32_t wave_incscan_max(int32_t v) {
  int32_t x = v;
  x = max(x, __builtin_amdgcn_update_dpp(0, x, 0x111, 0xf, 0xf, true));
  x = max(x, __builtin_amdgcn_update_dpp(0, x, 0x112, 0xf, 0xf, true));
  x = max(x, __builtin_amdgcn_update_dpp(0, x, 0x114, 0xf, 0xf, true));
  x = max(x, __builtin_amdgcn_update_dpp(0, x, 0x118, 0xf, 0xf, true));
  x = max(x, __builtin_amdgcn_update_dpp(0, x, 0x142, 0xa, 0xf, false));
  x = max(x, __builtin_amdgcn_update_dpp(0, x, 0x143, 0xc, 0xf, false));
  return x;
}
template <int NT>
__device__ __forceinline__ int32_t block_exscan_n(int32_t v, int32_t* total) {
  __shared__ int32_t wsum[NT / 64];
  const int lane = threadIdx.x & 63, wid = threadIdx.x >> 6;
  const int32_t x = wave_incscan(v);
  if (lane == 63) wsum[wid] = x;
  __syncthreads();
  int32_t base = 0, tot = 0;
#pragma unroll
  for (int w = 0; w < NT / 64; w++) {
    int32_t s = wsum[w];
    if (w < wid) base += s;
    tot += s;
  }
  __syncthreads();
  *total = tot;
  return base + x - v;
}
__device__ __forceinline__ int32_t block_exscan(int32_t v, int32_t* total) {
  return block_exscan_n<GPX_BLOCK>(v, total);
}


__device__ __forceinline__ int32_t tile_of_block(int32_t ntiles) {
  const int32_t per = (ntiles + 7) >> 3;
  return (int32_t)(blockIdx.x & 7) * per + (int32_t)(blockIdx.x >> 3);
}

__device__ __forceinline__ void bucket_count(int32_t* lds, int32_t b) {
  const unsigned long long act = __ballot(1);
  const int32_t b0 = __builtin_amdgcn_readfirstlane(b);
  if (__ballot(b == b0) == act) {
    if ((int)__lane_id() == __ffsll((long long)act) - 1) atomicAdd(&lds[b0], (int32_t)__popcll(act));
  } else {
    atomicAdd(&lds[b], 1);
  }
}
__device__ __forceinline__ int32_t bucket_take(int32_t* lds, int32_t b) {
  const unsigned long long act = __ballot(1);
  const int32_t b0 = __builtin_amdgcn_readfirstlane(b);
  if (__ballot(b == b0) == act) {
    const int lane = (int)__lane_id();
    const int leader = __ffsll((long long)act) - 1;
    const int32_t rank = (int32_t)__popcll(act & ((1ull << lane) - 1ull));
    int32_t base = 0;
    if (lane == leader) base = atomicAdd(&lds[b0], (int32_t)__popcll(act));
    return __shfl(base, leader, 64) + rank;
  }
  return atomicAdd(&lds[b], 1);
}

template <bool VEC>
__device__ __forceinline__ int32_t tile_histogram(int32_t n, int64_t base,
                                                  const int32_t* __restrict__ gidx, int32_t G,
                                                  int32_t shift, int32_t* lds, int32_t g_base, int32_t g_end) {
  int32_t bad = 0;
  const uint32_t span = (uint32_t)(g_end - g_base);
  auto one = [&](int32_t g) {
    if ((uint32_t)(g - g_base) < span)
      bucket_count(lds, (g - g_base) >> shift);
    else if ((uint32_t)g >= (uint32_t)G)
      bad++;
  };
  if (VEC) {
#pragma unroll
    for (int j = 0; j < GPX_TILE_VECS; j++) {
      const int64_t i0 = base + (int64_t)(j * GPX_FBLOCK + threadIdx.x) * 4;
      if (i0 + 3 < n) {
        const I4 g4 = *(const I4*)(gidx + i0);
        const int32_t gg[4] = {g4.x, g4.y, g4.z, g4.w};
#pragma unroll
        for (int q = 0; q < 4; q++) one(gg[q]);
      } else {
        for (int q = 0; q < 4; q++)
          if (i0 + q < n) one(gidx[i0 + q]);
      }
    }
// ... 422 lines not shown
    if (done >= c) return false;
    unsigned long long k;
    if (c <= 4)
      k = done == 0 ? k0 : (done == 1 ? k1 : (done == 2 ? k2 : k3));
    else
      k = keys[done];
    cur = (uint32_t)k;
    const int32_t* p = pay + (int64_t)cur * rs;
    out.idx = (int32_t)(k >> 32);
    out.a = p[0];
    out.b = p[fs];
    out.c = p[2 * fs];
    out.bnum = p[3 * fs];
    out.bcoord = p[4 * fs];
    done++;
    return true;
  }
  __device__ __forceinline__ void emit(int32_t slot, int32_t x, int32_t y, int32_t z, int32_t kind) {
    int32_t* p = pay + (int64_t)cur * rs;
    p[0] = slot;
    p[fs] = x;
    p[2 * fs] = y;
    p[3 * fs] = z;
    p[4 * fs] = kind;
    keys[nout++] = cur;
  }
  __device__ __forceinline__ void emit_at(uint32_t where, int32_t slot, int32_t x, int32_t y, int32_t z,
                                          int32_t kind) {
    int32_t* p = pay + (int64_t)where * rs;
    p[0] = slot;
    p[fs] = x;
    p[2 * fs] = y;
    p[3 * fs] = z;
    p[4 * fs] = kind;
    keys[nout++] = where;
  }
};

template <int KMAX>
__device__ __forceinline__ int32_t median_minus(const int32_t (&ns)[KMAX], int32_t k) {
  if (KMAX >= 3 && k == 3) {
    const int32_t lo = ns[0] < ns[1] ? ns[0] : ns[1], hi = ns[0] < ns[1] ? ns[1] : ns[0];
    const int32_t m = hi < ns[2] ? hi : ns[2];
    return lo > m ? lo : m;
  }
  const int32_t target = (k % 2 == 0) ? (k / 2 - 1) : (k / 2);
  int32_t res = 0;
#pragma unroll
  for (int j = 0; j < KMAX; j++) {
    if (j < k) {
      int32_t r = 0;
#pragma unroll
      for (int i = 0; i < KMAX; i++)
        if (i < k) r += (ns[i] < ns[j]) || (ns[i] == ns[j] && i < j);
      if (r == target) res = ns[j];
    }
  }
  return res;
}


__device__ __forceinline__ void bucket_emit(const DevScratch& X, const BucketView& bv) {
  __syncthreads();
  const int32_t b = blockIdx.x;
  const int32_t boff = X.bucket_off[b];
  const int32_t nt = (int32_t)blockDim.x;
  const int32_t per = X.gb / nt;
  int32_t s = 0;
  for (int32_t q = 0; q < per; q++) s += bv.lcnt[threadIdx.x * per + q];
  int32_t tot;
  int32_t ex = block_exscan_rt(s, &tot);
  Out* dst = X.o_rec + boff;
  const int32_t g0 = b << X.shift;
  for (int32_t q = 0; q < per; q++) {
    const int32_t l = threadIdx.x * per + q;
    const int32_t d = bv.lcnt[l];
    const unsigned long long* kk = bv.keys + bv.loff[l];
    for (int32_t t = 0; __any(t < d); t++) {
      int32_t pos = -1;
      I4 lo = mk4(0, 0, 0, 0), hi = mk4(0, 0, 0, 0);
      if (t < d) {
        const int32_t* p = bv.pay + (int64_t)(uint32_t)kk[t] * bv.rs;
        pos = ex + t;
        lo = mk4(g0 + l, p[0], p[bv.fs], p[2 * bv.fs]);
        hi = mk4(p[3 * bv.fs], p[4 * bv.fs], 0, 0);
      }
      store_rec_pair(dst, pos, lo, hi);
    }
    ex += d;
  }
  if (threadIdx.x == 0) X.bucket_nout[b] = tot;
}

__device__ __forceinline__ int32_t emit_base(const DevScratch& X, int32_t* total_out,
                                             unsigned long long* acc) {
  const int32_t b = blockIdx.x;
  int32_t before = 0;
  for (int32_t t = threadIdx.x; t < b; t += GPX_BLOCK) before += X.bucket_nout[t];
  int32_t pre;
  block_exscan(before, &pre);
  if (b == (int32_t)gridDim.x - 1 && threadIdx.x == 0) {
    const int32_t tot = pre + X.bucket_nout[b];
    if (total_out) *total_out = tot;
    if (acc) atomicAdd(acc, (unsigned long long)tot);
  }
  return pre;
}

__global__ __launch_bounds__(GPX_BLOCK) void k_emit_dec(
    DevScratch X, int32_t* __restrict__ d_gidx, int32_t* __restrict__ d_slot,
    int32_t* __restrict__ d_bnum, int32_t* __restrict__ d_bcoord, int32_t* __restrict__ d_median,
    uint8_t* __restrict__ d_kind, int32_t* total_out, unsigned long long* acc) {
  const int32_t out0 = emit_base(X, total_out, acc);
  const int32_t nd = X.bucket_nout[blockIdx.x];
  const Out* src = X.o_rec + X.bucket_off[blockIdx.x];
  for (int32_t t = threadIdx.x; t < nd; t += GPX_BLOCK) {
    const Out r = src[t];
    d_gidx[out0 + t] = r.gidx;
    d_slot[out0 + t] = r.slot;
    d_bnum[out0 + t] = r.x;
    d_bcoord[out0 + t] = r.y;
    d_median[out0 + t] = r.z;
    d_kind[out0 + t] = (uint8_t)r.kind;
  }
}

__global__ __launch_bounds__(GPX_BLOCK) void k_emit_runs(DevScratch X, int32_t* __restrict__ x_gidx,
                                                        int32_t* __restrict__ x_first,
                                                        int32_t* __restrict__ x_count,
                                                        int32_t* total_out) {
  if (*X.unsorted != X.epoch) return;
  const int32_t out0 = emit_base(X, total_out, nullptr);
  const int32_t nd = X.bucket_nout[blockIdx.x];
  const Out* src = X.o_rec + X.bucket_off[blockIdx.x];
  for (int32_t t = threadIdx.x; t < nd; t += GPX_BLOCK) {
    const Out r = src[t];
    x_gidx[out0 + t] = r.gidx;
    x_first[out0 + t] = r.x;
    x_count[out0 + t] = r.y;
  }
}

template <int KMAX>
struct CoordPre {
  uint32_t gf;
  int32_t my_bnum, my_bcoord, next, pcount;
  int32_t mem[KMAX], ns[KMAX];
  uint32_t pe;
  int32_t pe_slot;
  bool have_pe;
};
template <int KMAX>
__device__ __forceinline__ void coord_preload(const DevState& S, int32_t g, CoordPre<KMAX>& P) {
  const int32_t G = S.G;
  P.gf = S.g_flags[g];
  P.my_bnum = S.c_bnum[g];
  P.my_bcoord = S.c_bcoord[g];
  P.next = S.c_next[g];
  P.pcount = S.c_pcount[g];
#pragma unroll
  for (int j = 0; j < KMAX; j++) {
    P.mem[j] = (j < S.kmax) ? S.members[(int64_t)j * G + g] : 0;
    P.ns[j] = (j < S.kmax) ? S.node_slots[(int64_t)j * G + g] : 0;
  }
  P.pe = 0;
  P.pe_slot = 0;
  P.have_pe = false;
}
template <int KMAX>
__device__ __forceinline__ void coord_preload_ring(const DevState& S, int32_t g, CoordPre<KMAX>& P) {
  P.pe_slot = jsub(P.next, 1);
  P.pe = S.p_ring[(int64_t)(P.pe_slot & (S.W - 1)) * S.G + g];
  P.have_pe = true;
}
template <int KMAX>
__device__ __forceinline__ void coord_preload_ring_at(const DevState& S, int32_t g, int32_t slot, CoordPre<KMAX>& P) {
  P.pe_slot = slot;
  P.pe = S.p_ring[(int64_t)(slot & (S.W - 1)) * S.G + g];
  P.have_pe = true;
}

template <int KMAX, class IT>
__device__ __forceinline__ void apply_ar_group(const DevState& S, const DevScratch& X, int32_t g,
                                               IT& it, uint8_t* __restrict__ status,
                                               const CoordPre<KMAX>& P) {
  const int32_t G = S.G;
  const uint32_t gf = P.gf;
  if (!(gf & GF_EXISTS) || (gf & GF_STOPPED)) {
    const uint8_t st = (gf & GF_EXISTS) ? GPX_S_STOPPED : GPX_S_NOGROUP;
    Rec r;
    unsigned long long nd = 0;
    while (it.next(r)) {
      if (status) status[r.idx] = st;
      nd++;
    }
    atomicAdd(&X.counters[2], nd);
    return;
  }
  const int32_t k = (int32_t)GF_K(gf);
  bool has_coord = (gf & GF_HASCOORD) != 0;
  const bool preparing = (gf & GF_PREPARING) != 0;
  const int32_t my_bnum = P.my_bnum, my_bcoord = P.my_bcoord;
  const int32_t next = P.next;
  int32_t pcount = P.pcount;
  const int32_t pcount0 = pcount;
  const int32_t Wm = S.W - 1;
  int32_t mem[KMAX], ns[KMAX];
#pragma unroll
  for (int j = 0; j < KMAX; j++) {
    mem[j] = (j < k) ? P.mem[j] : 0;
    ns[j] = (j < k) ? P.ns[j] : 0;
  }
  bool ns_dirty = false;
  int64_t pc_off = P.have_pe ? ((int64_t)(P.pe_slot & Wm) * G + g) : -1;
  uint32_t pc_val = P.pe;
  bool pc_dirty = false;
  auto pr_load = [&](int64_t off) -> uint32_t {
    if (off != pc_off) {
      if (pc_dirty) S.p_ring[pc_off] = pc_val;
      pc_val = S.p_ring[off];
      pc_off = off;
      pc_dirty = false;
    }
    return pc_val;
  };
  auto pr_store = [&](uint32_t v) {
    pc_val = v;
    pc_dirty = true;
  };
  Rec r;
  while (it.next(r)) {
    const int32_t slot = r.a, acc = r.b, maxcp = r.c;
    if (!has_coord) continue;
    const int32_t cmp = ballot_cmp(r.bnum, r.bcoord, my_bnum, my_bcoord);
    const int32_t d = jsub(next, slot);
    const bool inwin = (d >= 1) && (d <= S.W) && !preparing;
    if (cmp > 0) {
      if (inwin) {
        const uint32_t e = pr_load((int64_t)(slot & Wm) * G + g);
        if (e & PR_PRESENT) {
          pr_store(0);
          pcount--;
          it.emit(slot, my_bnum, my_bcoord, -1, GPX_D_PREEMPTED);
        }
      }
      if (pcount == 0) has_coord = false;
    } else if (cmp == 0 && !preparing) {
      int32_t midx = -1;
#pragma unroll
      for (int q = 0; q < KMAX; q++) {
        if (q < k && mem[q] == acc) {
          midx = q;
          if (ns[q] < maxcp) {
            ns[q] = maxcp;
            ns_dirty = true;
          }
        }
      }
      if (inwin) {
        uint32_t e = pr_load((int64_t)(slot & Wm) * G + g);
        if (e & PR_PRESENT) {
          if (midx >= 0) e |= (1u << midx);
          if (__popc(e & 0xffffu) > k / 2) {
            pr_store(0);
            pcount--;
            it.emit(slot, my_bnum, my_bcoord, median_minus<KMAX>(ns, k), GPX_D_DECISION);
          } else {
            pr_store(e);
          }
        }
      }
    }
  }
  if (pc_dirty) S.p_ring[pc_off] = pc_val;
  if (ns_dirty) {
#pragma unroll
    for (int q = 0; q < KMAX; q++)
      if (q < k) S.node_slots[(int64_t)q * G + g] = ns[q];
  }
  if (pcount != pcount0) S.c_pcount[g] = pcount;
  if (!has_coord && (gf & GF_HASCOORD)) S.g_flags[g] = gf & ~(GF_HASCOORD | GF_PREPARING);
}

template <int KMAX>
struct SteadyGroup {
  int32_t mem[KMAX], ns[KMAX];
  int32_t k, pcount, pcount0;
  uint32_t e, e0;
  bool ns_dirty;
  static __device__ __forceinline__ bool group_ok(const CoordPre<KMAX>& P) {
    return (P.gf & (GF_EXISTS | GF_STOPPED | GF_HASCOORD | GF_PREPARING)) == (GF_EXISTS | GF_HASCOORD);
  }
  static __device__ __forceinline__ bool slot_ok(const DevState& S, const CoordPre<KMAX>& P, int32_t s0) {
    const int32_t d = jsub(P.next, s0);
    return d >= 1 && d <= S.W;
  }
  __device__ __forceinline__ void init(const DevState& S, int32_t g, const CoordPre<KMAX>& P, int32_t s0) {
    k = (int32_t)GF_K(P.gf);
#pragma unroll
    for (int j = 0; j < KMAX; j++) {
      mem[j] = (j < k) ? P.mem[j] : 0;
      ns[j] = (j < k) ? P.ns[j] : 0;
    }
    const int64_t off = (int64_t)(s0 & (S.W - 1)) * S.G + g;
    e0 = (P.have_pe && s0 == jsub(P.next, 1)) ? P.pe : S.p_ring[off];
    e = e0;
    pcount = pcount0 = P.pcount;
    ns_dirty = false;
  }
  __device__ __forceinline__ bool vote(int32_t acc, int32_t maxcp, int32_t* median) {
    int32_t midx = -1;
#pragma unroll
    for (int q = 0; q < KMAX; q++) {
      if (q < k && mem[q] == acc) {
        midx = q;
        if (ns[q] < maxcp) {
          ns[q] = maxcp;
          ns_dirty = true;
        }
      }
    }
    if (e & PR_PRESENT) {
      if (midx >= 0) e |= (1u << midx);
      if (__popc(e & 0xffffu) > k / 2) {
        *median = median_minus<KMAX>(ns, k);
        e = 0;
        pcount--;
        return true;
      }
    }
    return false;
  }
  __device__ __forceinline__ void finish(const DevState& S, int32_t g, int32_t s0) {
    if (e != e0) S.p_ring[(int64_t)(s0 & (S.W - 1)) * S.G + g] = e;
    if (ns_dirty) {
#pragma unroll
      for (int q = 0; q < KMAX; q++)
        if (q < k) S.node_slots[(int64_t)q * S.G + g] = ns[q];
    }
    if (pcount != pcount0) S.c_pcount[g] = pcount;
  }
};


struct AccState {
  int32_t slot, bnum, bcoord, gc;
  bool stopped;
};

#define AF_MASK 0xffu
#define CF_SHIFT 8
#define CF_MASK 0xff00u
struct AccView {
  I4* ring;
  int64_t G;
  int32_t g;
  int32_t w0, x0, y0, z0, f0;
  int32_t w1, x1, y1, z1, f1;
  __device__ __forceinline__ void init(const DevState& S, int32_t g_) {
    ring = S.acc_ring;
    G = S.G;
    g = g_;
    w0 = w1 = -1;
    x0 = y0 = z0 = f0 = 0;
    x1 = y1 = z1 = f1 = 0;
  }
  __device__ __forceinline__ void preset(int32_t w, const I4& v) {
    w0 = w;
    x0 = v.x;
    y0 = v.y;
    z0 = v.z;
    f0 = v.w;
  }
  __device__ __forceinline__ void put(int32_t w, const I4& v) {
    const bool in0 = w == w0 || w0 < 0;
    w0 = in0 ? w : w0;
    x0 = in0 ? v.x : x0;
    y0 = in0 ? v.y : y0;
    z0 = in0 ? v.z : z0;
    f0 = in0 ? v.w : f0;
    w1 = in0 ? w1 : w;
    x1 = in0 ? x1 : v.x;
    y1 = in0 ? y1 : v.y;
    z1 = in0 ? z1 : v.z;
    f1 = in0 ? f1 : v.w;
  }
  __device__ __forceinline__ I4 rd(int32_t w) {
    const bool h0 = w == w0, h1 = w == w1;
    I4 v = mk4(h0 ? x0 : x1, h0 ? y0 : y1, h0 ? z0 : z1, h0 ? f0 : f1);
    if (!(h0 || h1)) {
      v = ring[(int64_t)w * G + g];
      put(w, v);
    }
    return v;
  }
  __device__ __forceinline__ void wr(int32_t w, const I4& v) {
    ring[(int64_t)w * G + g] = v;
    put(w, v);
  }
  __device__ __forceinline__ void wr_flags(int32_t w, int32_t f) {
    ((int32_t*)&ring[(int64_t)w * G + g])[3] = f;
    f0 = (w == w0) ? f : f0;
    f1 = (w == w1 && w != w0) ? f : f1;
  }
};

__device__ __forceinline__ void acc_gc(const DevState& S, AccView& V, AccState& a, int32_t gcSlot) {
  if (jsub(a.slot, gcSlot) <= 0) gcSlot = jsub(a.slot, 1);
  const int32_t delta = jsub(gcSlot, a.gc);
  const bool far = jsub(a.slot, gcSlot) > INT32_MAX - 2 * S.W;
  if (delta > 0) {
    const int32_t Wm = S.W - 1;
    if (delta >= S.W || far) {
      for (int32_t w = 0; w < S.W; w++) {
        const I4 e = V.rd(w);
        if ((e.w & RF_PRESENT) && jsub(e.x, gcSlot) <= 0) V.wr_flags(w, e.w & ~(int32_t)AF_MASK);
      }
    } else {
      for (int32_t s = (int32_t)((uint32_t)a.gc + 1u);; s = (int32_t)((uint32_t)s + 1u)) {
        const I4 e = V.rd(s & Wm);
        if ((e.w & RF_PRESENT) && e.x == s) V.wr_flags(s & Wm, e.w & ~(int32_t)AF_MASK);
        if (s == gcSlot) break;
      }
    }
    a.gc = gcSlot;
  }
  if (far && jsub(gcSlot, a.slot) < 0) {
    for (int32_t w = 0; w < S.W; w++) {
      const I4 e = V.rd(w);
      if ((((uint32_t)e.w >> CF_SHIFT) & RF_PRESENT) && jsub(gcSlot, S.com_ring[(int64_t)w * S.G + V.g].x) > 0)
        V.wr_flags(w, e.w & ~(int32_t)CF_MASK);
    }
  }
}

struct Dec {
  int32_t bnum, bcoord, slot, median;
  bool has_value, stop;
};

__device__ __forceinline__ bool acc_reconstruct(const DevState& S, AccView& V, int32_t g, int32_t slot,
                                                Dec* out) {
  const int32_t w = slot & (S.W - 1);
  const I4 ar = V.rd(w);
  const uint32_t cf = ((uint32_t)ar.w >> CF_SHIFT) & 0xffu;
  const uint32_t af = (uint32_t)ar.w & AF_MASK;
  const I4 cr = S.com_ring[(int64_t)w * S.G + g];
  const bool committed = (cf & RF_PRESENT) && cr.x == slot;
  const bool hasv = (cf & RF_HASVALUE) != 0;
  const bool acc_ok = (af & RF_PRESENT) && ar.x == slot && ballot_cmp(ar.y, ar.z, cr.y, cr.z) == 0;
  Dec d;
  d.bnum = hasv ? cr.y : ar.y;
  d.bcoord = hasv ? cr.z : ar.z;
  d.slot = slot;
  d.median = cr.w;
  d.has_value = true;
  d.stop = ((hasv ? cf : af) & RF_STOP) != 0;
  *out = d;
  return committed && (hasv || acc_ok);
}

__device__ __forceinline__ int32_t acc_eec(const DevState& S, AccView& V, int32_t g, AccState& a,
                                           const Dec& d) {
  int32_t count = 0;
  const int32_t Wm = S.W - 1;
  const bool from_disk = (S.flags & GPX_F_ACCEPTS_FROM_DISK) != 0;
  while (!a.stopped) {
    acc_gc(S, V, a, d.median);
    bool direct = false;
    if (jsub(d.slot, a.slot) >= 0) {
      const int32_t wd = d.slot & Wm;
      const I4 e = V.rd(wd);
      const uint32_t cf = ((uint32_t)e.w >> CF_SHIFT) & 0xffu;
      bool same = false;
      if (cf & RF_PRESENT) same = S.com_ring[(int64_t)wd * S.G + g].x == d.slot;
      if (!same || !(cf & RF_HASVALUE)) {
        if (d.slot == a.slot && d.has_value) {
          direct = true;
          if (cf) V.wr_flags(wd, e.w & ~(int32_t)CF_MASK);
        } else {
          S.com_ring[(int64_t)wd * S.G + g] = mk4(d.slot, d.bnum, d.bcoord, d.median);
          const uint32_t nf = RF_PRESENT | (d.has_value ? RF_HASVALUE : 0u) | (d.stop ? RF_STOP : 0u);
          V.wr_flags(wd, (int32_t)(((uint32_t)e.w & ~CF_MASK) | (nf << CF_SHIFT)));
        }
      }
    }
    Dec nx = d;
    const int32_t wx = a.slot & Wm;
    if (!direct) {
      const I4 e2 = V.rd(wx);
      if (!(((uint32_t)e2.w >> CF_SHIFT) & RF_PRESENT)) break;
      nx = Dec{0, 0, 0, 0, false, false};
      if (!acc_reconstruct(S, V, g, a.slot, &nx)) break;
// ... 100 lines not shown
  AccState a;
  AccView V;
  acc_begin(S, g, pre, gf, a, V);
  const bool exists = (gf & GF_EXISTS) != 0;
  const AccState a0 = a;
  const int32_t Wm = S.W - 1;
  unsigned long long n_drop = 0;
  Rec r;
  while (it.next(r)) {
    const int32_t slot = r.a, median = r.b, ix = r.idx;
    const bool stop = (r.c & GPX_A_STOP) != 0;
    if (!exists || a.stopped) {
      put_reply(ix, 0, 0, 0, 0, r_bnum, r_bcoord, r_maxcp, r_flags, r_packed);
      status[ix] = exists ? GPX_S_STOPPED : GPX_S_NOGROUP;
      n_drop++;
      continue;
    }
    const int32_t w = slot & Wm;
    const I4 ar = V.rd(w);
    const bool live = (ar.w & RF_PRESENT) != 0;
    const bool have_prev = live && ar.x == slot;
    const bool ballot_ok = ballot_cmp(r.bnum, r.bcoord, a.bnum, a.bcoord) >= 0;
    const bool will_store = ballot_ok && jsub(slot, a.gc) > 0;
    if (will_store && live && ar.x != slot) {
      put_reply(ix, 0, 0, 0, 0, r_bnum, r_bcoord, r_maxcp, r_flags, r_packed);
      status[ix] = GPX_S_WINDOW;
      n_drop++;
      continue;
    }
    if (ballot_ok) {
      a.bnum = r.bnum;
      a.bcoord = r.bcoord;
      if (will_store)
        V.wr(w, mk4(slot, r.bnum, r.bcoord,
                    (int32_t)(((uint32_t)ar.w & CF_MASK) | RF_PRESENT | (stop ? (uint32_t)RF_STOP : 0u))));
    }
    acc_gc(S, V, a, median);
    const int32_t rep_bnum = a.bnum, rep_bcoord = a.bcoord, rep_maxcp = jsub(a.slot, 1);
    const bool to_log = ballot_cmp(r.bnum, r.bcoord, a.bnum, a.bcoord) >= 0 &&
                        jsub(slot, a.gc) > 0 &&
                        (!have_prev || ballot_cmp(ar.y, ar.z, r.bnum, r.bcoord) < 0);
    put_reply(ix, rep_bnum, rep_bcoord, rep_maxcp, (to_log ? GPX_R_TOLOG : 0) | (will_store ? GPX_R_STORED : 0),
              r_bnum, r_bcoord, r_maxcp, r_flags, r_packed);
    Dec rd = Dec{0, 0, 0, 0, false, false};
    if ((((uint32_t)V.rd(w).w >> CF_SHIFT) & RF_PRESENT) && acc_reconstruct(S, V, g, slot, &rd)) {
      const int32_t first = a.slot;
      const int32_t cnt_exec = acc_eec(S, V, g, a, rd);
      if (cnt_exec > 0) {
        it.emit(0, first, cnt_exec, 0, 1);
      }
    }
  }
  if (exists) acc_store(S, g, gf, a, a0);
  if (n_drop) atomicAdd(&X.counters[2], n_drop);
}

__global__ __launch_bounds__(1024) void k_bucket_accept(
    DevState S, DevScratch X, int32_t* __restrict__ r_bnum, int32_t* __restrict__ r_bcoord,
    int32_t* __restrict__ r_maxcp, uint8_t* __restrict__ r_flags, uint8_t* __restrict__ status) {
  extern __shared__ __attribute__((aligned(16))) int32_t lds[];
  BucketView bv;
  if (*X.unsorted != X.epoch) return;
  if (!bucket_prepare(X, lds, &bv, []() {})) return;
  const int32_t g0 = blockIdx.x << X.shift;
  for (int32_t l = threadIdx.x; l < X.gb; l += (int32_t)blockDim.x) {
    const int32_t c = bv.lcnt[l];
    int32_t nout = 0;
    if (c != 0 && g0 + l < S.G) {
      GroupIter it;
      it.init(bv, l, c);
      apply_accept_group(S, X, g0 + l, it, r_bnum, r_bcoord, r_maxcp, r_flags, status);
      nout = it.nout;
    }
    bv.lcnt[l] = nout;
  }
  bucket_emit(X, bv);
}

template <class IT>
__device__ __forceinline__ void apply_commit_group(const DevState& S, const DevScratch& X,
                                                   int32_t g, IT& it,
                                                   uint8_t* __restrict__ status, const AccPre pre = acc_nopre()) {
  uint32_t gf;
  AccState a;
  AccView V;
  acc_begin(S, g, pre, gf, a, V);
  const bool exists = (gf & GF_EXISTS) != 0;
  const AccState a0 = a;
  const int32_t Wm = S.W - 1;
  unsigned long long n_drop = 0;
  Rec r;
  while (it.next(r)) {
    const int32_t slot = r.a, median = r.b, kind = r.c, ix = r.idx;
    if (!exists || a.stopped) {
      status[ix] = exists ? GPX_S_STOPPED : GPX_S_NOGROUP;
      n_drop++;
      continue;
    }
    if (jsub(slot, a.slot) >= S.W) {
      status[ix] = GPX_S_WINDOW;
      n_drop++;
      continue;
    }
    Dec d = Dec{0, 0, 0, 0, false, false};
    if (kind & GPX_C_HASVALUE) {
      d = Dec{r.bnum, r.bcoord, slot, median, true, (kind & GPX_C_STOP) != 0};
    } else {
      const I4 ar = V.rd(slot & Wm);
      if ((ar.w & RF_PRESENT) && ar.x == slot && ballot_cmp(ar.y, ar.z, r.bnum, r.bcoord) == 0)
        d = Dec{ar.y, ar.z, slot, median, true, (ar.w & RF_STOP) != 0};
      else
        d = Dec{r.bnum, r.bcoord, slot, median, false, false};
    }
    const int32_t first = a.slot;
    const int32_t cnt_exec = acc_eec(S, V, g, a, d);
    if (cnt_exec > 0) {
      it.emit(0, first, cnt_exec, 0, 1);
    }
  }
  if (exists) acc_store(S, g, gf, a, a0);
  if (n_drop) atomicAdd(&X.counters[2], n_drop);
}

__global__ __launch_bounds__(1024) void k_bucket_commit(DevState S, DevScratch X,
                                                        uint8_t* __restrict__ status) {
  extern __shared__ __attribute__((aligned(16))) int32_t lds[];
  BucketView bv;
  if (*X.unsorted != X.epoch) return;
  if (!bucket_prepare(X, lds, &bv, []() {})) return;
  const int32_t g0 = blockIdx.x << X.shift;
  for (int32_t l = threadIdx.x; l < X.gb; l += (int32_t)blockDim.x) {
    const int32_t c = bv.lcnt[l];
    int32_t nout = 0;
    if (c != 0 && g0 + l < S.G) {
      GroupIter it;
      it.init(bv, l, c);
      apply_commit_group(S, X, g0 + l, it, status);
      nout = it.nout;
    }
    bv.lcnt[l] = nout;
  }
  bucket_emit(X, bv);
}

template <int KMAX>
struct ProposePre {
  uint32_t gf;
  int32_t a_bnum, a_bcoord, my_bnum, my_bcoord, next, pcount;
  int32_t ns[KMAX];
  uint32_t pe_prev, pe_cur;
};
template <int KMAX>
__device__ __forceinline__ void propose_preload(const DevState& S, int32_t g, ProposePre<KMAX>& P) {
  const int32_t G = S.G;
  P.gf = S.g_flags[g];
  P.a_bnum = S.a_bnum[g];
  P.a_bcoord = S.a_bcoord[g];
  P.my_bnum = S.c_bnum[g];
  P.my_bcoord = S.c_bcoord[g];
  P.next = S.c_next[g];
  P.pcount = S.c_pcount[g];
#pragma unroll
  for (int q = 0; q < KMAX; q++) P.ns[q] = (q < S.kmax) ? S.node_slots[(int64_t)q * G + g] : 0;
}
template <int KMAX>
__device__ __forceinline__ void propose_preload_ring(const DevState& S, int32_t g,
                                                     ProposePre<KMAX>& P) {
  const int32_t Wm = S.W - 1;
  P.pe_prev = S.p_ring[(int64_t)(jsub(P.next, 1) & Wm) * S.G + g];
  P.pe_cur = S.p_ring[(int64_t)(P.next & Wm) * S.G + g];
}

struct OneRec {
  int32_t idx, a, c, done;
  __device__ __forceinline__ bool next(Rec& out) {
    if (done) return false;
    out.idx = idx;
    out.a = a;
    done = 1;
    return true;
  }
};

template <int KMAX, class IT>
__device__ __forceinline__ void apply_propose_group(
    const DevState& S, const DevScratch& X, int32_t g, IT& it, int32_t* __restrict__ o_slot,
    int32_t* __restrict__ o_bnum, int32_t* __restrict__ o_bcoord, int32_t* __restrict__ o_median,
    uint8_t* __restrict__ status, const ProposePre<KMAX>& P, const int64_t* __restrict__ handle) {
  const int32_t G = S.G;
  const uint32_t gf = P.gf;
  const bool preparing = (gf & GF_PREPARING) != 0;
  const bool exists = (gf & GF_EXISTS) != 0, stopped = (gf & GF_STOPPED) != 0;
  const int32_t k = (int32_t)GF_K(gf);
  const int32_t a_bnum = exists ? P.a_bnum : 0, a_bcoord = exists ? P.a_bcoord : 0;
  const int32_t my_bnum = exists ? P.my_bnum : 0, my_bcoord = exists ? P.my_bcoord : 0;
  const bool coord_ok = exists && (gf & GF_HASCOORD) &&
                        ballot_cmp(my_bnum, my_bcoord, a_bnum, a_bcoord) >= 0;
  int32_t next = coord_ok ? P.next : 0;
  const int32_t next0 = next;
  int32_t pcount = coord_ok ? P.pcount : 0;
  int32_t ns[KMAX];
#pragma unroll
  for (int q = 0; q < KMAX; q++) ns[q] = (coord_ok && q < k) ? P.ns[q] : 0;
  const int32_t median = coord_ok ? median_minus<KMAX>(ns, k) : 0;
  const int32_t Wm = S.W - 1;
  uint32_t pe_prev = P.pe_prev, pe_cur = P.pe_cur;
  unsigned long long n_drop = 0;
  Rec r;
  while (it.next(r)) {
    const int32_t ix = r.idx;
    const bool stop = r.a != 0;
    int32_t st = GPX_S_OK, ob = 0, oc = 0;
    if (!exists || stopped) {
      st = exists ? GPX_S_STOPPED : GPX_S_NOGROUP;
      n_drop++;
    } else if (!coord_ok) {
      ob = a_bnum;
      oc = a_bcoord;
      st = GPX_S_FORWARD;
    } else if ((pe_prev & PR_PRESENT) && (pe_prev & PR_STOP)) {
      st = GPX_S_REFUSED;
    } else if (pe_cur & PR_PRESENT) {
      st = GPX_S_WINDOW;
      n_drop++;
    }
    if (st != GPX_S_OK) {
      o_slot[ix] = 0;
      o_bnum[ix] = ob;
      o_bcoord[ix] = oc;
      o_median[ix] = 0;
      status[ix] = (uint8_t)st;
      continue;
    }
    const uint32_t e = PR_PRESENT | (stop ? PR_STOP : 0u);
    S.p_ring[(int64_t)(next & Wm) * G + g] = e;
    pcount++;
    o_slot[ix] = next;
    o_bnum[ix] = my_bnum;
    o_bcoord[ix] = my_bcoord;
    o_median[ix] = preparing ? 0 : median;
    if (preparing) {
      S.p_handle[(int64_t)(next & Wm) * G + g] = handle ? handle[ix] : 0;
      status[ix] = GPX_S_PREACTIVE;
    }
    next = (int32_t)((uint32_t)next + 1u);
    pe_prev = e;
    if (it.done < it.c) pe_cur = S.p_ring[(int64_t)(next & Wm) * G + g];
  }
  if (coord_ok && next != next0) {
    S.c_next[g] = next;
    S.c_pcount[g] = pcount;
  }
  if (n_drop) atomicAdd(&X.counters[2], n_drop);
}

template <int KMAX>
__global__ __launch_bounds__(1024) void k_bucket_propose(
    DevState S, DevScratch X, int32_t* __restrict__ o_slot, int32_t* __restrict__ o_bnum,
    int32_t* __restrict__ o_bcoord, int32_t* __restrict__ o_median, uint8_t* __restrict__ status,
    const int64_t* __restrict__ handle) {
  extern __shared__ __attribute__((aligned(16))) int32_t lds[];
  BucketView bv;
  if (*X.unsorted != X.epoch) {
    if (threadIdx.x == 0) X.bucket_tot[blockIdx.x] = 0;
    return;
  }
  const int32_t g0 = blockIdx.x << X.shift;
  const int32_t nb_ = X.bucket_off[blockIdx.x + 1] - X.bucket_off[blockIdx.x];
  const bool pre = (int32_t)blockDim.x == X.gb && 2 * nb_ >= X.gb;
  const int32_t gme = g0 + (int32_t)threadIdx.x;
  ProposePre<KMAX> P;
  if (pre && gme < S.G) propose_preload<KMAX>(S, gme, P);
  if (!bucket_prepare(X, lds, &bv, [&]() {
        if (pre && gme < S.G) propose_preload_ring<KMAX>(S, gme, P);
      }))
    return;
  for (int32_t l = threadIdx.x; l < X.gb; l += (int32_t)blockDim.x) {
    const int32_t c = bv.lcnt[l];
    if (c == 0 || g0 + l >= S.G) continue;
    GroupIter it;
    it.init(bv, l, c);
    if (!pre) {
      propose_preload<KMAX>(S, g0 + l, P);
      propose_preload_ring<KMAX>(S, g0 + l, P);
    }
    apply_propose_group<KMAX, GroupIter>(S, X, g0 + l, it, o_slot, o_bnum, o_bcoord, o_median, status, P, handle);
  }
}


#define GPX_OC_BLOCK 256
template <bool STRICT>
__global__ __launch_bounds__(GPX_OC_BLOCK) void k_order_check(int32_t n, const int32_t* __restrict__ gidx,
                                                           int32_t G, DevScratch X,
                                                           uint8_t* __restrict__ status,
                                                           int32_t* __restrict__ zero, int32_t nzero) {
  const int64_t i0 = ((int64_t)blockIdx.x * GPX_OC_BLOCK + threadIdx.x) * 8;
  if (zero && i0 / 8 < nzero) zero[i0 / 8] = 0;
  bool bad = false;
  if (i0 < n) {
    int32_t g[9];
    const bool full = i0 + 8 < n;
    if (full && !((uintptr_t)gidx & 15)) {
      const I4 a = *(const I4*)(gidx + i0), b = *(const I4*)(gidx + i0 + 4);
      g[0] = a.x; g[1] = a.y; g[2] = a.z; g[3] = a.w;
      g[4] = b.x; g[5] = b.y; g[6] = b.z; g[7] = b.w;
      g[8] = gidx[i0 + 8];
    } else {
#pragma unroll
      for (int q = 0; q < 9; q++) g[q] = (i0 + q < n) ? gidx[i0 + q] : INT32_MAX;
    }
    unsigned long long stw = 0;
#pragma unroll
    for (int q = 0; q < 8; q++) {
      if (i0 + q < n) {
        const bool oob = (uint32_t)g[q] >= (uint32_t)G;
        bad |= oob || (i0 + q + 1 < n && (STRICT ? g[q] >= g[q + 1] : g[q] > g[q + 1]));
        if (oob) stw |= (unsigned long long)GPX_S_NOGROUP << (8 * q);
      }
    }
    if (!status) {
    } else if (full && !((uintptr_t)status & 7)) {
      *(unsigned long long*)(status + i0) = stw;
    } else {
      for (int q = 0; q < 8; q++)
        if (i0 + q < n) status[i0 + q] = (uint8_t)(stw >> (8 * q));
    }
  }
  if (__syncthreads_or(bad) && threadIdx.x == 0) atomicMax(X.unsorted, X.epoch);
}

template <int KMAX>
__global__ __launch_bounds__(GPX_BLOCK) void k_propose_direct(
    DevState S, DevScratch X, int32_t n, const int32_t* __restrict__ gidx,
    const uint8_t* __restrict__ is_stop, int32_t* __restrict__ o_slot, int32_t* __restrict__ o_bnum,
    int32_t* __restrict__ o_bcoord, int32_t* __restrict__ o_median, uint8_t* __restrict__ status,
    const int64_t* __restrict__ handle, int32_t refuse) {
  const int32_t i = blockIdx.x * GPX_BLOCK + threadIdx.x;
  if (*X.unsorted == X.epoch) {
    if (refuse && i < n) {
      o_slot[i] = 0;
      o_bnum[i] = 0;
      o_bcoord[i] = 0;
      o_median[i] = 0;
      status[i] = GPX_S_UNORDERED;
    }
    return;
  }
  if (i >= n) return;
  const int32_t g = gidx[i];
  ProposePre<KMAX> P;
  propose_preload<KMAX>(S, g, P);
  propose_preload_ring<KMAX>(S, g, P);
  OneRec it;
  it.idx = i;
  it.a = is_stop ? (int32_t)(is_stop[i] & 1) : 0;
  it.c = 1;
  it.done = 0;
  apply_propose_group<KMAX, OneRec>(S, X, g, it, o_slot, o_bnum, o_bcoord, o_median, status, P, handle);
}

template <bool STRICT>
__device__ __forceinline__ uint32_t small_batch_first_bad(int32_t n, const int32_t* __restrict__ gidx, int32_t G) {
  __shared__ uint32_t s_first_bad;
  if (threadIdx.x == 0) s_first_bad = 0xffffffffu;
  uint32_t mine = 0xffffffffu;
  const int32_t B = (int32_t)blockDim.x, t = (int32_t)threadIdx.x;
  for (int32_t r0 = 0; r0 < n; r0 += 16 * B) {
    int32_t gg[16], gp[16];
#pragma unroll
    for (int k = 0; k < 16; k++) {
      const int32_t ic = min(r0 + k * B + t, n - 1);
      gg[k] = gidx[ic];
      gp[k] = gidx[max(ic - 1, 0)];
    }
#pragma unroll
    for (int k = 15; k >= 0; k--) {
      const int32_t i = r0 + k * B + t;
      const bool viol = i < n && ((uint32_t)gg[k] >= (uint32_t)G || (i > 0 && (STRICT ? gp[k] >= gg[k] : gp[k] > gg[k])));
      mine = viol ? min(mine, (uint32_t)i) : mine;
    }
  }
  if (__syncthreads_or(mine != 0xffffffffu)) {
    if (mine != 0xffffffffu) atomicMin(&s_first_bad, mine);
    __syncthreads();
  }
  return s_first_bad;
}
template <bool STRICT>
__device__ __forceinline__ bool small_batch_ordered(int32_t n, const int32_t* __restrict__ gidx, int32_t G) {
  return small_batch_first_bad<STRICT>(n, gidx, G) == 0xffffffffu;
}

template <int KMAX>
__global__ __launch_bounds__(GPX_BLOCK) void k_propose_small(
    DevState S, DevScratch X, int32_t n, const int32_t* __restrict__ gidx,
    const uint8_t* __restrict__ is_stop, int32_t* __restrict__ o_slot, int32_t* __restrict__ o_bnum,
    int32_t* __restrict__ o_bcoord, int32_t* __restrict__ o_median, uint8_t* __restrict__ status,
    const int64_t* __restrict__ handle, int32_t refuse) {
  const int32_t i = blockIdx.x * GPX_BLOCK + threadIdx.x;
  const int32_t g = i < n ? gidx[i] : -1;
  ProposePre<KMAX> P;
  if ((uint32_t)g < (uint32_t)S.G) {
    propose_preload<KMAX>(S, g, P);
// ... 26 lines not shown
struct PrepOut {
  int32_t n;
  int32_t *r_bnum, *r_bcoord, *r_gc;
  uint8_t* r_flags;
  unsigned long long* p_mask;
  int32_t *p_slot, *p_bnum, *p_bcoord;
  uint8_t* status;
};
__global__ __launch_bounds__(1024) void k_bucket_prepare(DevState S, DevScratch X, PrepOut O) {
  extern __shared__ __attribute__((aligned(16))) int32_t lds[];
  BucketView bv;
  if (!bucket_prepare(X, lds, &bv, []() {})) return;
  const int32_t g0 = blockIdx.x << X.shift;
  for (int32_t l = threadIdx.x; l < X.gb; l += (int32_t)blockDim.x) {
    const int32_t c = bv.lcnt[l];
    const int32_t g = g0 + l;
    if (c == 0 || g >= S.G) continue;
    GroupIter it;
    it.init(bv, l, c);
    const uint32_t gf = S.g_flags[g];
    const bool exists = (gf & GF_EXISTS) != 0, stopped = (gf & GF_STOPPED) != 0;
    int32_t bn = exists ? S.a_bnum[g] : 0, bc = exists ? S.a_bcoord[g] : 0;
    const int32_t bn0 = bn, bc0 = bc;
    const int32_t gc = exists ? S.a_gc[g] : 0;
    unsigned long long n_drop = 0;
    Rec r;
    while (it.next(r)) {
      const int32_t ix = r.idx, first = r.a;
      O.r_bnum[ix] = 0;
      O.r_bcoord[ix] = 0;
      O.r_gc[ix] = 0;
      O.r_flags[ix] = 0;
      O.p_mask[ix] = 0;
      if (!exists || stopped) {
        O.status[ix] = exists ? GPX_S_STOPPED : GPX_S_NOGROUP;
        n_drop++;
        continue;
      }
      const int32_t pn = bn, pc = bc;
      if (ballot_cmp(r.bnum, r.bcoord, bn, bc) > 0) {
        bn = r.bnum;
        bc = r.bcoord;
      }
      const bool nack = ballot_cmp(bn, bc, r.bnum, r.bcoord) > 0;
      unsigned long long mask = 0;
      if (!nack) {
        for (int32_t w = 0; w < S.W; w++) {
          const int64_t o = (int64_t)w * S.G + g;
          const I4 a = S.acc_ring[o];
          if (!(a.w & RF_PRESENT)) continue;
          if (jsub(a.x, first) < 0) continue;
          mask |= 1ull << w;
          const int64_t q = (int64_t)w * O.n + ix;
          O.p_slot[q] = a.x;
          O.p_bnum[q] = a.y;
          O.p_bcoord[q] = a.z;
        }
      }
      O.r_bnum[ix] = bn;
      O.r_bcoord[ix] = bc;
      const int32_t fm1 = jsub(first, 1);
      O.r_gc[ix] = jsub(gc, fm1) < 0 ? fm1 : gc;
      O.r_flags[ix] = (uint8_t)((nack ? GPX_P_NACK : 0) | (ballot_cmp(pn, pc, bn, bc) < 0 ? GPX_P_TOLOG : 0));
      O.p_mask[ix] = mask;
    }
    if (exists && (bn != bn0 || bc != bc0)) {
      S.a_bnum[g] = bn;
      S.a_bcoord[g] = bc;
    }
    if (n_drop) atomicAdd(&X.counters[2], n_drop);
  }
}

__global__ __launch_bounds__(1024) void k_bucket_reqbatch(DevState S, DevScratch X, int32_t max_bytes,
                                                          int32_t max_size,
                                                          int32_t* __restrict__ leader) {
  extern __shared__ __attribute__((aligned(16))) int32_t lds[];
  BucketView bv;
  if (!bucket_prepare(X, lds, &bv, []() {})) return;
  const int32_t g0 = blockIdx.x << X.shift;
  for (int32_t l = threadIdx.x; l < X.gb; l += (int32_t)blockDim.x) {
    const int32_t c = bv.lcnt[l];
    int32_t nout = 0;
    if (c != 0 && g0 + l < S.G) {
      GroupIter it;
      it.init(bv, l, c);
      int32_t head = -1, count = 0, stop = 0;
      uint32_t head_cur = 0;
      long long bytes = 0, size = 0;
      Rec r;
      while (it.next(r)) {
        const long long est = r.a, w = r.b;
        bool fresh = head < 0;
        if (!fresh) {
          if (bytes + est > max_bytes || size + w > max_size) {
            it.emit_at(head_cur, head, count, (int32_t)bytes, (int32_t)size, stop);
            fresh = true;
          }
        }
        if (fresh) {
          head = r.idx;
          head_cur = it.cur;
          count = 1;
          bytes = est;
          size = w;
          stop = r.c & 1;
        } else {
          count++;
          bytes += est;
          size += w;
          stop |= r.c & 1;
        }
        leader[r.idx] = head;
      }
      if (head >= 0) it.emit_at(head_cur, head, count, (int32_t)bytes, (int32_t)size, stop);
      nout = it.nout;
    }
    bv.lcnt[l] = nout;
  }
  bucket_emit(X, bv);
}

__global__ __launch_bounds__(GPX_BLOCK) void k_fill_i32(int32_t n, int32_t v, int32_t* __restrict__ a) {
  const int32_t i = blockIdx.x * GPX_BLOCK + threadIdx.x;
  if (i < n) a[i] = v;
}

#define GPX_MAX_NODE_LIST 16
struct NodeLists {
  int32_t n_down, n_long;
  int32_t down[GPX_MAX_NODE_LIST], longdead[GPX_MAX_NODE_LIST];
};
__global__ __launch_bounds__(GPX_BLOCK) void k_election_scan(DevState S, int32_t n,
                                                            const int32_t* __restrict__ gidx,
                                                            NodeLists L, int32_t force,
                                                            uint8_t* __restrict__ run,
                                                            int32_t* __restrict__ p_bnum,
                                                            int32_t* __restrict__ p_first,
                                                            uint8_t* __restrict__ status) {
  const int32_t i = blockIdx.x * GPX_BLOCK + threadIdx.x;
  if (i >= n) return;
  const int32_t g = gidx ? gidx[i] : i;
  run[i] = GPX_RUN_NO;
  p_bnum[i] = 0;
  p_first[i] = 0;
  if ((uint32_t)g >= (uint32_t)S.G || !(S.g_flags[g] & GF_EXISTS)) {
    status[i] = GPX_S_NOGROUP;
    return;
  }
  status[i] = GPX_S_OK;
  const uint32_t gf = S.g_flags[g];
  const int32_t k = (int32_t)GF_K(gf);
  const int32_t bn = S.a_bnum[g], bc = S.a_bcoord[g];
  const bool have = (gf & GF_HASCOORD) && ballot_cmp(S.c_bnum[g], S.c_bcoord[g], bn, bc) >= 0;
  bool down = false, longdead = false;
  for (int32_t q = 0; q < L.n_down; q++) down |= L.down[q] == bc;
  for (int32_t q = 0; q < L.n_long; q++) longdead |= L.longdead[q] == bc;
  int32_t next = INT32_MIN;
  bool member = false;
  for (int32_t q = 0; q < k; q++)
    if (S.members[(int64_t)q * S.G + g] == bc) {
      next = S.members[(int64_t)((q + 1) % k) * S.G + g];
      member = true;
    }
  int32_t why = GPX_RUN_NO;
  if (!have) {
    if (bc == S.my_id)
      why = GPX_RUN_MINE;
    else if (down && member && next == S.my_id)
      why = GPX_RUN_NEXT;
    else if (down && longdead)
      why = GPX_RUN_LONGDEAD;
  }
  if (why == GPX_RUN_NO && force) why = GPX_RUN_FORCED;
  if (why != GPX_RUN_NO) {
    run[i] = (uint8_t)why;
    p_bnum[i] = (int32_t)((uint32_t)bn + 1u);
    p_first[i] = S.a_slot[g];
  }
}

__global__ __launch_bounds__(GPX_BLOCK) void k_gap_scan(DevState S, int32_t n,
                                                       const int32_t* __restrict__ gidx,
                                                       int32_t threshold, int32_t sync_mode,
                                                       int32_t size_limit,
                                                       int32_t* __restrict__ first_slot,
                                                       int32_t* __restrict__ max_committed,
                                                       unsigned long long* __restrict__ missing,
                                                       uint8_t* __restrict__ should_sync,
                                                       uint8_t* __restrict__ status) {
  const int32_t i = blockIdx.x * GPX_BLOCK + threadIdx.x;
  if (i >= n) return;
  const int32_t g = gidx[i];
  first_slot[i] = 0;
  max_committed[i] = 0;
  missing[i] = 0;
  should_sync[i] = 0;
  if ((uint32_t)g >= (uint32_t)S.G || !(S.g_flags[g] & GF_EXISTS)) {
    status[i] = GPX_S_NOGROUP;
    return;
  }
  const uint32_t gf = S.g_flags[g];
  const int32_t slot = S.a_slot[g];
  first_slot[i] = slot;
  const bool stopped = (gf & GF_STOPPED) != 0;
  int32_t maxc = jsub(slot, 1);
  if (!stopped) {
    bool any = false;
    int32_t last = INT32_MIN, wrapmax = maxc;
    for (int32_t w = 0; w < S.W; w++) {
      const int64_t o = (int64_t)w * S.G + g;
      if (!(((uint32_t)S.acc_ring[o].w >> CF_SHIFT) & RF_PRESENT)) continue;
      const int32_t key = S.com_ring[o].x;
      any = true;
      last = key > last ? key : last;
    }
    if (any && last == INT32_MAX) {
      for (int32_t w = 0; w < S.W; w++) {
        const int64_t o = (int64_t)w * S.G + g;
        if ((((uint32_t)S.acc_ring[o].w >> CF_SHIFT) & RF_PRESENT) && jsub(S.com_ring[o].x, wrapmax) > 0) wrapmax = S.com_ring[o].x;
      }
      last = wrapmax;
    }
    if (any) maxc = last;
  }
  max_committed[i] = maxc;
  const int32_t gap = jsub(maxc, slot);
  const bool nontrivial = gap >= threshold / 100;
  const bool small_thr = threshold <= 1;
  const bool sync = (gap >= threshold) || ((slot == 0 || slot == 1) && (nontrivial || small_thr)) ||
                    (nontrivial && sync_mode == GPX_SYNC_TO_PAUSE) || sync_mode == GPX_SYNC_FORCE;
  should_sync[i] = sync ? 1 : 0;
  status[i] = stopped ? GPX_S_STOPPED : GPX_S_OK;
  if (stopped) return;
  unsigned long long m = 0;
  const int32_t limit = (int32_t)((uint32_t)slot + (uint32_t)size_limit);
  const int32_t Wm = S.W - 1;
  int32_t j = 0;
  for (int32_t s = slot; jsub(s, maxc) < 0 && jsub(s, limit) < 0 && j < 64;
       s = (int32_t)((uint32_t)s + 1u), j++) {
    const int64_t o = (int64_t)(s & Wm) * S.G + g;
    const I4 ae = S.acc_ring[o];
    const uint32_t cf = ((uint32_t)ae.w >> CF_SHIFT) & 0xffu;
    const bool have = (cf & RF_PRESENT) && S.com_ring[o].x == s;
    const bool acc = (ae.w & RF_PRESENT) && ae.x == s;
    if (!have || (!(cf & RF_HASVALUE) && !acc)) m |= 1ull << j;
  }
  missing[i] = m;
}

#define GPX_NAME_ROW_STRIDE 160
#define GPX_NAME_ROW_EXISTS 5
#define GPX_NAME_ROW_VERSION 8
#define GPX_NAME_ROW_SLOT 144
#define GPX_NAME_BUCKET_BYTES 128
#define GPX_NAME_BUCKET_KEYS 32
#define GPX_NAME_PAYLOAD_BYTES 24
struct NameCopies {
  uint8_t* rows;
  uint8_t* tab;
  __device__ __forceinline__ void set(int32_t g, bool exists, bool set_version, int32_t version) const {
    if (!rows) return;
    uint8_t* nr = rows + (int64_t)g * GPX_NAME_ROW_STRIDE;
    if (set_version) *(int32_t*)(nr + GPX_NAME_ROW_VERSION) = version;
    nr[GPX_NAME_ROW_EXISTS] = exists ? 1 : 0;
    if (nr[4] != 0) {
      const int32_t s = *(const int32_t*)(nr + GPX_NAME_ROW_SLOT);
      if (s >= 0) {
        uint8_t* e = tab + (int64_t)(s >> 2) * GPX_NAME_BUCKET_BYTES + GPX_NAME_BUCKET_KEYS + (s & 3) * GPX_NAME_PAYLOAD_BYTES;
        if (set_version) *(int32_t*)(e + 4) = version;
        e[1] = exists ? 1 : 0;
      }
    }
  }
};

__global__ __launch_bounds__(GPX_BLOCK) void k_group_create(DevState S, int32_t n,
                                                           const int32_t* __restrict__ gidx,
                                                           const int32_t* __restrict__ members,
                                                           const uint8_t* __restrict__ kk,
                                                           const gpx_hri* __restrict__ rows,
                                                           uint8_t* __restrict__ status,
                                                           NameCopies names) {
  int32_t i = blockIdx.x * GPX_BLOCK + threadIdx.x;
  if (i >= n) return;
  const int32_t g = gidx[i];
  const int32_t k = kk[i];
  if ((uint32_t)g >= (uint32_t)S.G || k < 1 || k > S.kmax) {
    status[i] = GPX_S_NOGROUP;
    return;
  }
  if (S.g_flags[g] & GF_EXISTS) {
    status[i] = GPX_S_EXISTS;
    return;
  }
  const gpx_hri r = rows[i];
  const bool coord = r.has_coord && r.coord_bcoord == S.my_id;
  S.g_version[g] = r.version;
  S.a_slot[g] = r.acc_slot;
  S.a_bnum[g] = r.acc_bnum;
  S.a_bcoord[g] = r.acc_bcoord;
  S.a_gc[g] = r.acc_gc_slot;
  S.c_bnum[g] = coord ? r.coord_bnum : 0;
  S.c_bcoord[g] = coord ? r.coord_bcoord : 0;
  S.c_next[g] = coord ? r.next_proposal_slot : 0;
  S.c_pcount[g] = 0;
  for (int32_t j = 0; j < S.kmax; j++) {
    S.members[(int64_t)j * S.G + g] = (j < k) ? members[(int64_t)i * S.kmax + j] : 0;
    S.node_slots[(int64_t)j * S.G + g] = (coord && j < k) ? r.node_slots[j] : 0;
  }
  for (int32_t w = 0; w < S.W; w++) {
    const int64_t o = (int64_t)w * S.G + g;
    S.p_ring[o] = 0;
    S.acc_ring[o] = mk4(0, 0, 0, 0);
  }
  S.g_flags[g] = GF_EXISTS | (coord ? GF_HASCOORD : 0u) | ((uint32_t)k << 8);
  names.set(g, true, true, r.version);
  status[i] = GPX_S_OK;
}

__device__ __forceinline__ void fill_hri_dev(const DevState& S, int32_t g, uint32_t gf,
                                             gpx_hri* out) {
  gpx_hri r;
  r.version = S.g_version[g];
  r.acc_slot = S.a_slot[g];
  r.acc_bnum = S.a_bnum[g];
  r.acc_bcoord = S.a_bcoord[g];
  r.acc_gc_slot = S.a_gc[g];
  const bool coord = (gf & GF_HASCOORD) != 0 && !(gf & GF_PREPARING);
  const int32_t k = (int32_t)GF_K(gf);
  r.has_coord = coord ? 1 : 0;
  r.coord_bnum = coord ? S.c_bnum[g] : 0;
  r.coord_bcoord = coord ? S.c_bcoord[g] : 0;
  r.next_proposal_slot = coord ? S.c_next[g] : -1;
  for (int32_t j = 0; j < GPX_KMAX_LIMIT; j++)
    r.node_slots[j] = (coord && j < k && j < S.kmax) ? S.node_slots[(int64_t)j * S.G + g] : 0;
  *out = r;
}

__global__ __launch_bounds__(GPX_BLOCK) void k_group_retire(DevState S, int32_t n,
                                                           const int32_t* __restrict__ gidx,
                                                           int32_t mode, gpx_hri* __restrict__ rows,
                                                           uint8_t* __restrict__ status,
                                                           NameCopies names) {
  int32_t i = blockIdx.x * GPX_BLOCK + threadIdx.x;
  if (i >= n) return;
  const int32_t g = gidx[i];
  gpx_hri zero = {};
  if (rows) rows[i] = zero;
  if ((uint32_t)g >= (uint32_t)S.G || !(S.g_flags[g] & GF_EXISTS)) {
    if (status) status[i] = GPX_S_NOGROUP;
    return;
  }
  const uint32_t gf = S.g_flags[g];
  if (mode == GPX_RETIRE_PAUSE) {
    bool caught = true;
    const bool from_disk = (S.flags & GPX_F_ACCEPTS_FROM_DISK) != 0;
    for (int32_t w = 0; w < S.W; w++) {
      const int64_t o = (int64_t)w * S.G + g;
      const int32_t fl = S.acc_ring[o].w;
      if (((uint32_t)fl >> CF_SHIFT) & RF_PRESENT) caught = false;
      if (!from_disk && (fl & RF_PRESENT)) caught = false;
    }
    if ((gf & GF_HASCOORD) && S.c_pcount[g] != 0) caught = false;
    if (!caught) {
      if (status) status[i] = GPX_S_BUSY;
      return;
    }
  }
  if (rows) fill_hri_dev(S, g, gf, &rows[i]);
  if (mode != 2) {
    S.g_flags[g] = 0;
    names.set(g, false, false, 0);
  }
  if (status) status[i] = GPX_S_OK;
}
```

Baseline: 12.42 billion decisions/s.

## Pack coordinator state into paired 8-byte rows and use 32-bit state offsets

```diff
diff --git a/gigapaxos_amd/csrc/gpx_ar16.hip.h b/gigapaxos_amd/csrc/gpx_ar16.hip.h
--- a/gigapaxos_amd/csrc/gpx_ar16.hip.h
+++ b/gigapaxos_amd/csrc/gpx_ar16.hip.h
@@ -366,15 +366,16 @@
   }
   if (fast) {
     if (OP == B16_AR) {
-      const int32_t G = S.G, k = (int32_t)GF_K(P.gf);
+      const int32_t k = (int32_t)GF_K(P.gf);
+      const uint32_t G = (uint32_t)S.G, ug = (uint32_t)g;
       int32_t mem[KMAX], ns[KMAX];
 #pragma unroll
       for (int j = 0; j < KMAX; j++) {
         mem[j] = (j < k) ? P.mem[j] : 0;
         ns[j] = (j < k) ? P.ns[j] : 0;
       }
-      const int64_t off = (int64_t)(s0 & (S.W - 1)) * G + g;
-      const uint32_t e0 = (P.have_pe && s0 == jsub(P.next, 1)) ? P.pe : S.p_ring[off];
+      const uint32_t off = (uint32_t)(s0 & (S.W - 1)) * G + ug;
+      const uint32_t e0 = (P.have_pe && s0 == jsub(P.next, 1)) ? P.pe : *at32(S.p_ring, off);
       uint32_t e = e0;
       int32_t pcount = P.pcount;
       bool ns_dirty = false;
@@ -416,13 +417,13 @@
           vote(i, p, (meta & V16_ESC) ? in.acceptor[idxA[p]] : (int32_t)(meta >> 16), cpA[p]);
         }
       }
-      if (e != e0) S.p_ring[off] = e;
+      if (e != e0) *at32(S.p_ring, off) = e;
       if (ns_dirty) {
 #pragma unroll
         for (int q = 0; q < KMAX; q++)
-          if (q < k) S.node_slots[(int64_t)q * G + g] = ns[q];
-      }
-      if (pcount != P.pcount) S.c_pcount[g] = pcount;
+          if (q < k) *at32(S.node_slots, (uint32_t)q * G + ug) = ns[q];
+      }
+      if (pcount != P.pcount) coord_put_pcount(S, ug, pcount);
     }
   } else {
     replay(it);
@@ -906,8 +907,7 @@
     DevScratch X, Stage16 O, int32_t* __restrict__ d_gidx, int32_t* __restrict__ d_slot,
     int32_t* __restrict__ d_bnum, int32_t* __restrict__ d_bcoord, int32_t* __restrict__ d_median,
     uint8_t* __restrict__ d_kind, int32_t* total_out, unsigned long long* acc, const int32_t* base_in,
-    int32_t* chain_out, int32_t* in_place = nullptr, int32_t nvotes = 0, const int32_t* __restrict__ c_bnum = nullptr,
-    const int32_t* __restrict__ c_bcoord = nullptr) {
+    int32_t* chain_out, int32_t* in_place = nullptr, int32_t nvotes = 0, BallotSrc c_hot = BallotSrc{nullptr, nullptr}) {
   if (X.gate && *X.unsorted != X.epoch) return;
   const bool placed = in_place && in_place[3] != (int32_t)X.epoch;
   if (placed && blockIdx.x != gridDim.x - 1) return;
@@ -935,8 +935,15 @@
     const int32_t g = O.gidx()[src + t];
     d_gidx[out0 + t] = g;
     d_slot[out0 + t] = O.slot()[src + t];
-    d_bnum[out0 + t] = c_bnum ? c_bnum[g] : O.bnum()[src + t];
-    d_bcoord[out0 + t] = c_bnum ? c_bcoord[g] : O.bcoord()[src + t];
+    int32_t bn, bc;
+    if (c_hot.a) {
+      c_hot.get(g, &bn, &bc);
+    } else {
+      bn = O.bnum()[src + t];
+      bc = O.bcoord()[src + t];
+    }
+    d_bnum[out0 + t] = bn;
+    d_bcoord[out0 + t] = bc;
     d_median[out0 + t] = O.median()[src + t];
     d_kind[out0 + t] = O.kind()[src + t];
   }
diff --git a/gigapaxos_amd/csrc/gpx_elect.hip.h b/gigapaxos_amd/csrc/gpx_elect.hip.h
--- a/gigapaxos_amd/csrc/gpx_elect.hip.h
+++ b/gigapaxos_amd/csrc/gpx_elect.hip.h
@@ -31,12 +31,14 @@
   const uint32_t gf = S.g_flags[g];
   const int32_t k = (int32_t)GF_K(gf);
   const bool has = (gf & GF_HASCOORD) != 0;
-  const int32_t cmp = has ? ballot_cmp(S.c_bnum[g], S.c_bcoord[g], bnum[i], S.my_id) : -1;
+  const int32_t cmp = has ? ballot_cmp(coord_row(S, (uint32_t)g).bnum, coord_row(S, (uint32_t)g).bcoord, bnum[i], S.my_id) : -1;
   if (!has || cmp < 0) {
-    S.c_bnum[g] = bnum[i];
-    S.c_bcoord[g] = S.my_id;
-    S.c_next[g] = S.a_slot[g];
-    S.c_pcount[g] = 0;
+    CHot h;
+    h.bnum = bnum[i];
+    h.bcoord = S.my_id;
+    h.next = S.a_slot[g];
+    h.pcount = 0;
+    coord_put(S, (uint32_t)g, h);
     S.c_wait[g] = 0;
     for (int32_t j = 0; j < k; j++) S.node_slots[(int64_t)j * S.G + g] = -1;
     for (int32_t w = 0; w < S.W; w++) {
@@ -85,7 +87,7 @@
         pk = GPX_POKE_PREPARE;
         hd = S.c_wait[g];
       } else {
-        const int32_t d = jsub(S.c_next[g], s);
+        const int32_t d = jsub(coord_row(S, (uint32_t)g).next, s);
         const uint32_t e = (d >= 1 && d <= S.W) ? S.p_ring[(int64_t)(s & (S.W - 1)) * S.G + g] : 0u;
         if (e & PR_PRESENT) {
           const int32_t k = (int32_t)GF_K(gf);
@@ -100,8 +102,8 @@
       }
       if (pk != GPX_POKE_NONE) {
         sl = s;
-        bn = S.c_bnum[g];
-        bc = S.c_bcoord[g];
+        bn = coord_row(S, (uint32_t)g).bnum;
+        bc = coord_row(S, (uint32_t)g).bcoord;
       }
     }
   }
@@ -156,8 +158,10 @@
   const bool exists = (gf & GF_EXISTS) != 0;
   const int32_t k = (int32_t)GF_K(gf);
   const bool had = exists && (gf & GF_HASCOORD);
-  const int32_t my_bnum = had ? S.c_bnum[g] : 0, my_bcoord = had ? S.c_bcoord[g] : 0;
-  int32_t next = had ? S.c_next[g] : 0, pcount = had ? S.c_pcount[g] : 0;
+  CHot h0 = {0, 0, 0, 0};
+  if (had) h0 = coord_row(S, (uint32_t)g);
+  const int32_t my_bnum = h0.bnum, my_bcoord = h0.bcoord;
+  int32_t next = h0.next, pcount = h0.pcount;
   uint32_t wait = (had && (gf & GF_PREPARING)) ? S.c_wait[g] : 0u;
   int32_t mem[KMAX], ns[KMAX];
 #pragma unroll
@@ -401,8 +405,7 @@
   }
   if (wait_dirty) S.c_wait[g] = wait;
   if (prop_dirty) {
-    S.c_next[g] = next;
-    S.c_pcount[g] = pcount;
+    coord_put_tail(S, (uint32_t)g, next, pcount);
   }
   if (gf != gf0) S.g_flags[g] = gf;
   if (n_drop) atomicAdd(&X.counters[2], n_drop);
diff --git a/gigapaxos_amd/csrc/gpx_engine.hip b/gigapaxos_amd/csrc/gpx_engine.hip
--- a/gigapaxos_amd/csrc/gpx_engine.hip
+++ b/gigapaxos_amd/csrc/gpx_engine.hip
@@ -589,6 +589,11 @@
   if (cfg->max_groups <= 0 || cfg->kmax < 1 || cfg->kmax > GPX_KMAX_LIMIT || cfg->max_batch <= 0)
     return GPX_EINVAL;
   if (cfg->window < 4 || cfg->window > 64 || (cfg->window & (cfg->window - 1))) return GPX_EINVAL;
+  if (!gpx_state_offsets32_ok(cfg->max_groups, cfg->window, cfg->kmax)) {
+    snprintf(g_err, sizeof(g_err), "max_groups %d x window %d x kmax %d: a state array of 4 GiB or more", cfg->max_groups,
+             cfg->window, cfg->kmax);
+    return GPX_EINVAL;
+  }
   int ndev = 0;
   hipError_t de = hipErrorNoDevice;
   const int attempts = access("/dev/kfd", F_OK) == 0 ? 15 : 1;
@@ -643,10 +648,17 @@
   A(S.a_bnum, G, true);
   A(S.a_bcoord, G, true);
   A(S.a_gc, G, true);
+#if GPX_CLAYOUT == 0
   A(S.c_bnum, G, true);
   A(S.c_bcoord, G, true);
   A(S.c_next, G, true);
   A(S.c_pcount, G, true);
+#elif GPX_CLAYOUT == 1
+  A(S.c_hot, G, true);
+#else
+  A(S.c_ballot, G, true);
+  A(S.c_prog, G, true);
+#endif
   A(S.members, K * G, true);
   A(S.node_slots, K * G, true);
   A(S.p_ring, W * G, true);
@@ -1199,7 +1211,7 @@
   }
   LAUNCH(e, "k_emit_dec16", k_emit_dec16, e->X.nbk, e->X, O, d_gidx, d_slot, d_bnum, d_bcoord, d_median_cp, d_kind, n_out,
          &e->X.counters[1], (const int32_t*)nullptr, (int32_t*)nullptr, ip_div ? A.ref : (int32_t*)nullptr, n,
-         ip_div ? (const int32_t*)e->S.c_bnum : (const int32_t*)nullptr, (const int32_t*)e->S.c_bcoord);
+         ip_div ? ballot_src(e->S) : BallotSrc{nullptr, nullptr});
 #ifdef GPX_TL_TRACE
   tl_trace_end(e);
 #endif
@@ -2689,12 +2701,20 @@
     }
     w.push_back((gf & GF_HASCOORD) ? 1 : 0);
     if (gf & GF_HASCOORD) {
-      int32_t next = 0;
-      HIPCHK(rd32(S.c_bnum, gidx, &v));
-      w.push_back(v);
-      HIPCHK(rd32(S.c_bcoord, gidx, &v));
-      w.push_back(v);
-      HIPCHK(rd32(S.c_next, gidx, &next));
+      CHot hot;
+#if GPX_CLAYOUT == 0
+      HIPCHK(rd32(S.c_bnum, gidx, &hot.bnum));
+      HIPCHK(rd32(S.c_bcoord, gidx, &hot.bcoord));
+      HIPCHK(rd32(S.c_next, gidx, &hot.next));
+#elif GPX_CLAYOUT == 1
+      HIPCHK(hipMemcpy(&hot, S.c_hot + gidx, sizeof(CHot), hipMemcpyDeviceToHost));
+#else
+      HIPCHK(hipMemcpy(&hot.bnum, S.c_ballot + gidx, 8, hipMemcpyDeviceToHost));
+      HIPCHK(hipMemcpy(&hot.next, S.c_prog + gidx, 8, hipMemcpyDeviceToHost));
+#endif
+      const int32_t next = hot.next;
+      w.push_back(hot.bnum);
+      w.push_back(hot.bcoord);
       w.push_back(next);
       for (int j = 0; j < k; j++) {
         HIPCHK(rd32(S.node_slots, (int64_t)j * S.G + gidx, &v));
diff --git a/gigapaxos_amd/csrc/gpx_kernels.hip.h b/gigapaxos_amd/csrc/gpx_kernels.hip.h
--- a/gigapaxos_amd/csrc/gpx_kernels.hip.h
+++ b/gigapaxos_amd/csrc/gpx_kernels.hip.h
@@ -89,13 +89,43 @@
 #define RF_STOP 2
 #define RF_HASVALUE 4
 
+struct __attribute__((aligned(16))) CHot {
+  int32_t bnum, bcoord, next, pcount;
+};
+struct __attribute__((aligned(8))) CHotTail {
+  int32_t next, pcount;
+};
+struct __attribute__((aligned(8))) CHotHead {
+  int32_t bnum, bcoord;
+};
+static_assert(sizeof(CHot) == 16 && offsetof(CHot, next) == 8 && sizeof(CHotTail) == 8, "c_hot row");
+#ifndef GPX_CLAYOUT
+#define GPX_CLAYOUT 2
+#endif
+
+template <class T>
+__device__ __forceinline__ T* at32(T* base, uint32_t i) {
+  return (T*)((char*)base + i * (uint32_t)sizeof(T));
+}
+__host__ __device__ inline bool gpx_state_offsets32_ok(int64_t G, int64_t W, int64_t kmax) {
+  const int64_t lim = (int64_t)1 << 32;
+  return G > 0 && W > 0 && kmax > 0 && G * 16 < lim && kmax * G * 4 < lim && W * G * 4 < lim;
+}
+
 struct DevState {
   int32_t G, kmax, W, my_id;
   uint32_t flags;
   uint32_t* g_flags;
   int32_t* g_version;
   int32_t *a_slot, *a_bnum, *a_bcoord, *a_gc;
+#if GPX_CLAYOUT == 0
   int32_t *c_bnum, *c_bcoord, *c_next, *c_pcount;
+#elif GPX_CLAYOUT == 1
+  CHot* c_hot;
+#else
+  CHotHead* c_ballot;
+  CHotTail* c_prog;
+#endif
   int32_t* members;
   int32_t* node_slots;
   uint32_t* p_ring;
@@ -107,6 +137,93 @@
   int64_t* p_handle;
 };
 #define CO_PRESENT 0x100
+
+__device__ __forceinline__ CHot coord_row(const DevState& S, uint32_t ug) {
+#if GPX_CLAYOUT == 0
+  CHot h;
+  h.bnum = *at32(S.c_bnum, ug);
+  h.bcoord = *at32(S.c_bcoord, ug);
+  h.next = *at32(S.c_next, ug);
+  h.pcount = *at32(S.c_pcount, ug);
+  return h;
+#elif GPX_CLAYOUT == 1
+  return *at32(S.c_hot, ug);
+#else
+  const CHotHead a = *at32(S.c_ballot, ug);
+  const CHotTail b = *at32(S.c_prog, ug);
+  CHot h;
+  h.bnum = a.bnum;
+  h.bcoord = a.bcoord;
+  h.next = b.next;
+  h.pcount = b.pcount;
+  return h;
+#endif
+}
+__device__ __forceinline__ void coord_put_tail(const DevState& S, uint32_t ug, int32_t next, int32_t pcount) {
+#if GPX_CLAYOUT == 0
+  *at32(S.c_next, ug) = next;
+  *at32(S.c_pcount, ug) = pcount;
+#else
+  CHotTail t;
+  t.next = next;
+  t.pcount = pcount;
+#if GPX_CLAYOUT == 1
+  *(CHotTail*)&at32(S.c_hot, ug)->next = t;
+#else
+  *at32(S.c_prog, ug) = t;
+#endif
+#endif
+}
+__device__ __forceinline__ void coord_put_pcount(const DevState& S, uint32_t ug, int32_t pcount) {
+#if GPX_CLAYOUT == 0
+  *at32(S.c_pcount, ug) = pcount;
+#elif GPX_CLAYOUT == 1
+  at32(S.c_hot, ug)->pcount = pcount;
+#else
+  at32(S.c_prog, ug)->pcount = pcount;
+#endif
+}
+__device__ __forceinline__ void coord_put(const DevState& S, uint32_t ug, const CHot& h) {
+#if GPX_CLAYOUT == 0
+  *at32(S.c_bnum, ug) = h.bnum;
+  *at32(S.c_bcoord, ug) = h.bcoord;
+  coord_put_tail(S, ug, h.next, h.pcount);
+#elif GPX_CLAYOUT == 1
+  *at32(S.c_hot, ug) = h;
+#else
+  CHotHead a;
+  a.bnum = h.bnum;
+  a.bcoord = h.bcoord;
+  *at32(S.c_ballot, ug) = a;
+  coord_put_tail(S, ug, h.next, h.pcount);
+#endif
+}
+struct BallotSrc {
+  const void *a, *b;
+  __device__ __forceinline__ void get(int32_t g, int32_t* bn, int32_t* bc) const {
+#if GPX_CLAYOUT == 0
+    *bn = ((const int32_t*)a)[g];
+    *bc = ((const int32_t*)b)[g];
+#elif GPX_CLAYOUT == 1
+    const CHotHead h = *(const CHotHead*)&((const CHot*)a)[g];
+    *bn = h.bnum;
+    *bc = h.bcoord;
+#else
+    const CHotHead h = ((const CHotHead*)a)[g];
+    *bn = h.bnum;
+    *bc = h.bcoord;
+#endif
+  }
+};
+inline BallotSrc ballot_src(const DevState& S) {
+#if GPX_CLAYOUT == 0
+  return BallotSrc{S.c_bnum, S.c_bcoord};
+#elif GPX_CLAYOUT == 1
+  return BallotSrc{S.c_hot, nullptr};
+#else
+  return BallotSrc{S.c_ballot, nullptr};
+#endif
+}
 
 struct DevScratch {
   int32_t shift, nbk, gb;
@@ -835,16 +952,17 @@
 };
 template <int KMAX>
 __device__ __forceinline__ void coord_preload(const DevState& S, int32_t g, CoordPre<KMAX>& P) {
-  const int32_t G = S.G;
-  P.gf = S.g_flags[g];
-  P.my_bnum = S.c_bnum[g];
-  P.my_bcoord = S.c_bcoord[g];
-  P.next = S.c_next[g];
-  P.pcount = S.c_pcount[g];
+  const uint32_t G = (uint32_t)S.G, ug = (uint32_t)g;
+  P.gf = *at32(S.g_flags, ug);
+  const CHot h = coord_row(S, ug);
+  P.my_bnum = h.bnum;
+  P.my_bcoord = h.bcoord;
+  P.next = h.next;
+  P.pcount = h.pcount;
 #pragma unroll
   for (int j = 0; j < KMAX; j++) {
-    P.mem[j] = (j < S.kmax) ? S.members[(int64_t)j * G + g] : 0;
-    P.ns[j] = (j < S.kmax) ? S.node_slots[(int64_t)j * G + g] : 0;
+    P.mem[j] = (j < S.kmax) ? *at32(S.members, (uint32_t)j * G + ug) : 0;
+    P.ns[j] = (j < S.kmax) ? *at32(S.node_slots, (uint32_t)j * G + ug) : 0;
   }
   P.pe = 0;
   P.pe_slot = 0;
@@ -853,13 +971,13 @@
 template <int KMAX>
 __device__ __forceinline__ void coord_preload_ring(const DevState& S, int32_t g, CoordPre<KMAX>& P) {
   P.pe_slot = jsub(P.next, 1);
-  P.pe = S.p_ring[(int64_t)(P.pe_slot & (S.W - 1)) * S.G + g];
+  P.pe = *at32(S.p_ring, (uint32_t)(P.pe_slot & (S.W - 1)) * (uint32_t)S.G + (uint32_t)g);
   P.have_pe = true;
 }
 template <int KMAX>
 __device__ __forceinline__ void coord_preload_ring_at(const DevState& S, int32_t g, int32_t slot, CoordPre<KMAX>& P) {
   P.pe_slot = slot;
-  P.pe = S.p_ring[(int64_t)(slot & (S.W - 1)) * S.G + g];
+  P.pe = *at32(S.p_ring, (uint32_t)(slot & (S.W - 1)) * (uint32_t)S.G + (uint32_t)g);
   P.have_pe = true;
 }
 
@@ -867,7 +985,7 @@
 __device__ __forceinline__ void apply_ar_group(const DevState& S, const DevScratch& X, int32_t g,
                                                IT& it, uint8_t* __restrict__ status,
                                                const CoordPre<KMAX>& P) {
-  const int32_t G = S.G;
+  const uint32_t G = (uint32_t)S.G, ug = (uint32_t)g;
   const uint32_t gf = P.gf;
   if (!(gf & GF_EXISTS) || (gf & GF_STOPPED)) {
     const uint8_t st = (gf & GF_EXISTS) ? GPX_S_STOPPED : GPX_S_NOGROUP;
@@ -895,13 +1013,13 @@
     ns[j] = (j < k) ? P.ns[j] : 0;
   }
   bool ns_dirty = false;
-  int64_t pc_off = P.have_pe ? ((int64_t)(P.pe_slot & Wm) * G + g) : -1;
+  uint32_t pc_off = P.have_pe ? ((uint32_t)(P.pe_slot & Wm) * G + ug) : ~0u;
   uint32_t pc_val = P.pe;
   bool pc_dirty = false;
-  auto pr_load = [&](int64_t off) -> uint32_t {
+  auto pr_load = [&](uint32_t off) -> uint32_t {
     if (off != pc_off) {
-      if (pc_dirty) S.p_ring[pc_off] = pc_val;
-      pc_val = S.p_ring[off];
+      if (pc_dirty) *at32(S.p_ring, pc_off) = pc_val;
+      pc_val = *at32(S.p_ring, off);
       pc_off = off;
       pc_dirty = false;
     }
@@ -920,7 +1038,7 @@
     const bool inwin = (d >= 1) && (d <= S.W) && !preparing;
     if (cmp > 0) {
       if (inwin) {
-        const uint32_t e = pr_load((int64_t)(slot & Wm) * G + g);
+        const uint32_t e = pr_load((uint32_t)(slot & Wm) * G + ug);
         if (e & PR_PRESENT) {
           pr_store(0);
           pcount--;
@@ -941,7 +1059,7 @@
         }
       }
       if (inwin) {
-        uint32_t e = pr_load((int64_t)(slot & Wm) * G + g);
+        uint32_t e = pr_load((uint32_t)(slot & Wm) * G + ug);
         if (e & PR_PRESENT) {
           if (midx >= 0) e |= (1u << midx);
           if (__popc(e & 0xffffu) > k / 2) {
@@ -955,13 +1073,13 @@
       }
     }
   }
-  if (pc_dirty) S.p_ring[pc_off] = pc_val;
+  if (pc_dirty) *at32(S.p_ring, pc_off) = pc_val;
   if (ns_dirty) {
 #pragma unroll
     for (int q = 0; q < KMAX; q++)
-      if (q < k) S.node_slots[(int64_t)q * G + g] = ns[q];
-  }
-  if (pcount != pcount0) S.c_pcount[g] = pcount;
+      if (q < k) *at32(S.node_slots, (uint32_t)q * G + ug) = ns[q];
+  }
+  if (pcount != pcount0) coord_put_pcount(S, ug, pcount);
   if (!has_coord && (gf & GF_HASCOORD)) S.g_flags[g] = gf & ~(GF_HASCOORD | GF_PREPARING);
 }
 
@@ -985,8 +1103,8 @@
       mem[j] = (j < k) ? P.mem[j] : 0;
       ns[j] = (j < k) ? P.ns[j] : 0;
     }
-    const int64_t off = (int64_t)(s0 & (S.W - 1)) * S.G + g;
-    e0 = (P.have_pe && s0 == jsub(P.next, 1)) ? P.pe : S.p_ring[off];
+    const uint32_t off = (uint32_t)(s0 & (S.W - 1)) * (uint32_t)S.G + (uint32_t)g;
+    e0 = (P.have_pe && s0 == jsub(P.next, 1)) ? P.pe : *at32(S.p_ring, off);
     e = e0;
     pcount = pcount0 = P.pcount;
     ns_dirty = false;
@@ -1015,13 +1133,14 @@
     return false;
   }
   __device__ __forceinline__ void finish(const DevState& S, int32_t g, int32_t s0) {
-    if (e != e0) S.p_ring[(int64_t)(s0 & (S.W - 1)) * S.G + g] = e;
+    const uint32_t G = (uint32_t)S.G, ug = (uint32_t)g;
+    if (e != e0) *at32(S.p_ring, (uint32_t)(s0 & (S.W - 1)) * G + ug) = e;
     if (ns_dirty) {
 #pragma unroll
       for (int q = 0; q < KMAX; q++)
-        if (q < k) S.node_slots[(int64_t)q * S.G + g] = ns[q];
-    }
-    if (pcount != pcount0) S.c_pcount[g] = pcount;
+        if (q < k) *at32(S.node_slots, (uint32_t)q * G + ug) = ns[q];
+    }
+    if (pcount != pcount0) coord_put_pcount(S, ug, pcount);
   }
 };
 
@@ -1428,23 +1547,25 @@
 };
 template <int KMAX>
 __device__ __forceinline__ void propose_preload(const DevState& S, int32_t g, ProposePre<KMAX>& P) {
-  const int32_t G = S.G;
-  P.gf = S.g_flags[g];
-  P.a_bnum = S.a_bnum[g];
-  P.a_bcoord = S.a_bcoord[g];
-  P.my_bnum = S.c_bnum[g];
-  P.my_bcoord = S.c_bcoord[g];
-  P.next = S.c_next[g];
-  P.pcount = S.c_pcount[g];
-#pragma unroll
-  for (int q = 0; q < KMAX; q++) P.ns[q] = (q < S.kmax) ? S.node_slots[(int64_t)q * G + g] : 0;
+  const uint32_t G = (uint32_t)S.G, ug = (uint32_t)g;
+  P.gf = *at32(S.g_flags, ug);
+  P.a_bnum = *at32(S.a_bnum, ug);
+  P.a_bcoord = *at32(S.a_bcoord, ug);
+  const CHot h = coord_row(S, ug);
+  P.my_bnum = h.bnum;
+  P.my_bcoord = h.bcoord;
+  P.next = h.next;
+  P.pcount = h.pcount;
+#pragma unroll
+  for (int q = 0; q < KMAX; q++) P.ns[q] = (q < S.kmax) ? *at32(S.node_slots, (uint32_t)q * G + ug) : 0;
 }
 template <int KMAX>
 __device__ __forceinline__ void propose_preload_ring(const DevState& S, int32_t g,
                                                      ProposePre<KMAX>& P) {
   const int32_t Wm = S.W - 1;
-  P.pe_prev = S.p_ring[(int64_t)(jsub(P.next, 1) & Wm) * S.G + g];
-  P.pe_cur = S.p_ring[(int64_t)(P.next & Wm) * S.G + g];
+  const uint32_t G = (uint32_t)S.G, ug = (uint32_t)g;
+  P.pe_prev = *at32(S.p_ring, (uint32_t)(jsub(P.next, 1) & Wm) * G + ug);
+  P.pe_cur = *at32(S.p_ring, (uint32_t)(P.next & Wm) * G + ug);
 }
 
 struct OneRec {
@@ -1463,7 +1584,7 @@
     const DevState& S, const DevScratch& X, int32_t g, IT& it, int32_t* __restrict__ o_slot,
     int32_t* __restrict__ o_bnum, int32_t* __restrict__ o_bcoord, int32_t* __restrict__ o_median,
     uint8_t* __restrict__ status, const ProposePre<KMAX>& P, const int64_t* __restrict__ handle) {
-  const int32_t G = S.G;
+  const uint32_t G = (uint32_t)S.G, ug = (uint32_t)g;
   const uint32_t gf = P.gf;
   const bool preparing = (gf & GF_PREPARING) != 0;
   const bool exists = (gf & GF_EXISTS) != 0, stopped = (gf & GF_STOPPED) != 0;
@@ -1509,23 +1630,22 @@
       continue;
     }
     const uint32_t e = PR_PRESENT | (stop ? PR_STOP : 0u);
-    S.p_ring[(int64_t)(next & Wm) * G + g] = e;
+    *at32(S.p_ring, (uint32_t)(next & Wm) * G + ug) = e;
     pcount++;
     o_slot[ix] = next;
     o_bnum[ix] = my_bnum;
     o_bcoord[ix] = my_bcoord;
     o_median[ix] = preparing ? 0 : median;
     if (preparing) {
-      S.p_handle[(int64_t)(next & Wm) * G + g] = handle ? handle[ix] : 0;
+      S.p_handle[(int64_t)(next & Wm) * S.G + g] = handle ? handle[ix] : 0;
       status[ix] = GPX_S_PREACTIVE;
     }
     next = (int32_t)((uint32_t)next + 1u);
     pe_prev = e;
-    if (it.done < it.c) pe_cur = S.p_ring[(int64_t)(next & Wm) * G + g];
+    if (it.done < it.c) pe_cur = *at32(S.p_ring, (uint32_t)(next & Wm) * G + ug);
   }
   if (coord_ok && next != next0) {
-    S.c_next[g] = next;
-    S.c_pcount[g] = pcount;
+    coord_put_tail(S, ug, next, pcount);
   }
   if (n_drop) atomicAdd(&X.counters[2], n_drop);
 }
@@ -1858,7 +1978,7 @@
   const uint32_t gf = S.g_flags[g];
   const int32_t k = (int32_t)GF_K(gf);
   const int32_t bn = S.a_bnum[g], bc = S.a_bcoord[g];
-  const bool have = (gf & GF_HASCOORD) && ballot_cmp(S.c_bnum[g], S.c_bcoord[g], bn, bc) >= 0;
+  const bool have = (gf & GF_HASCOORD) && ballot_cmp(coord_row(S, (uint32_t)g).bnum, coord_row(S, (uint32_t)g).bcoord, bn, bc) >= 0;
   bool down = false, longdead = false;
   for (int32_t q = 0; q < L.n_down; q++) down |= L.down[q] == bc;
   for (int32_t q = 0; q < L.n_long; q++) longdead |= L.longdead[q] == bc;
@@ -2007,10 +2127,12 @@
   S.a_bnum[g] = r.acc_bnum;
   S.a_bcoord[g] = r.acc_bcoord;
   S.a_gc[g] = r.acc_gc_slot;
-  S.c_bnum[g] = coord ? r.coord_bnum : 0;
-  S.c_bcoord[g] = coord ? r.coord_bcoord : 0;
-  S.c_next[g] = coord ? r.next_proposal_slot : 0;
-  S.c_pcount[g] = 0;
+  CHot h;
+  h.bnum = coord ? r.coord_bnum : 0;
+  h.bcoord = coord ? r.coord_bcoord : 0;
+  h.next = coord ? r.next_proposal_slot : 0;
+  h.pcount = 0;
+  coord_put(S, (uint32_t)g, h);
   for (int32_t j = 0; j < S.kmax; j++) {
     S.members[(int64_t)j * S.G + g] = (j < k) ? members[(int64_t)i * S.kmax + j] : 0;
     S.node_slots[(int64_t)j * S.G + g] = (coord && j < k) ? r.node_slots[j] : 0;
@@ -2036,9 +2158,10 @@
   const bool coord = (gf & GF_HASCOORD) != 0 && !(gf & GF_PREPARING);
   const int32_t k = (int32_t)GF_K(gf);
   r.has_coord = coord ? 1 : 0;
-  r.coord_bnum = coord ? S.c_bnum[g] : 0;
-  r.coord_bcoord = coord ? S.c_bcoord[g] : 0;
-  r.next_proposal_slot = coord ? S.c_next[g] : -1;
+  const CHot h = coord_row(S, (uint32_t)g);
+  r.coord_bnum = coord ? h.bnum : 0;
+  r.coord_bcoord = coord ? h.bcoord : 0;
+  r.next_proposal_slot = coord ? h.next : -1;
   for (int32_t j = 0; j < GPX_KMAX_LIMIT; j++)
     r.node_slots[j] = (coord && j < k && j < S.kmax) ? S.node_slots[(int64_t)j * S.G + g] : 0;
   *out = r;
@@ -2068,7 +2191,7 @@
       if (((uint32_t)fl >> CF_SHIFT) & RF_PRESENT) caught = false;
       if (!from_disk && (fl & RF_PRESENT)) caught = false;
     }
-    if ((gf & GF_HASCOORD) && S.c_pcount[g] != 0) caught = false;
+    if ((gf & GF_HASCOORD) && coord_row(S, (uint32_t)g).pcount != 0) caught = false;
     if (!caught) {
       if (status) status[i] = GPX_S_BUSY;
       return;
```

New measurement: 12.21 billion decisions/s, median of 2. -1.7%, worse.
